# Quantco/tabmat

Hardware: AMD Instinct MI355X
Metric: SplitMatrix.sandwich GFLOP/s + effective HBM GB/s, 10M×1k mixed (higher is better)
Workload: dtype f64; 1 GPU; SplitMatrix.sandwich: dense128 + csr512@5% + cats(256,96,32), 10000000 rows/GPU, p=1024, float64 (BASELINE configs[3]); rows_per_gpu=10000000, p=1024, launch=eager, collective=none

## Files before the change

### tabmat_amd/csrc/cat_multi.hip

```cpp
#include <algorithm>
#include <type_traits>

#include "common.hpp"
#include "reduce.hpp"

namespace tmh {

constexpr int MAX_CATS = 16;
struct CatSet {
    const int32_t *codes[MAX_CATS];
    int ncol[MAX_CATS];
    int drop[MAX_CATS];
    int off[MAX_CATS];
    int n_cats;
    int total;
};

__host__ __device__ constexpr size_t tile_lds_bytes(size_t nel) { return ((nel * sizeof(lds_acc_t) + 15) / 16) * 16; }

__device__ __forceinline__ void zero_tile(lds_acc_t *tile, int nel) {
    for (int b = threadIdx.x; b < nel; b += blockDim.x) tile[b] = 0.0;
}

__device__ __forceinline__ unsigned char *scratch_behind_tile(unsigned char *smem, int nel) {
    return smem + tile_lds_bytes((size_t)nel);
}

template <typename F>
__device__ __forceinline__ F *workgroup_slice(F *ws, int64_t stride) {
    return ws + ((int64_t)blockIdx.y * gridDim.x + blockIdx.x) * stride;
}

template <typename F>
__device__ __forceinline__ void store_tile(const lds_acc_t *tile, int rows, int tstr, int cols, F *__restrict__ dst) {
    if (tstr == cols) {
        for (int b = threadIdx.x; b < rows * cols; b += blockDim.x) dst[b] = (F)tile[b];
    } else {
        for (int b = threadIdx.x; b < rows * cols; b += blockDim.x) dst[b] = (F)tile[(b / cols) * tstr + (b % cols)];
    }
}

__device__ __forceinline__ int level_of(const int32_t *codes, int drop, int64_t row) { return codes[row] - drop; }

constexpr int PACKED_BITS = 10;
constexpr int PACKED_NONE = (1 << PACKED_BITS) - 1;
__device__ __forceinline__ int packed_field(unsigned pk, int c) { return (int)((pk >> (PACKED_BITS * c)) & (unsigned)PACKED_NONE); }

template <typename F, int TJ, int NC>
__global__ __launch_bounds__(1024) void multi_cat_dense_c_kernel(
    CatSet cs, const F *__restrict__ d, const F *__restrict__ M, int64_t n, int64_t m,
    int64_t rows_per_block, F *__restrict__ ws, int64_t stride) {
    extern __shared__ __attribute__((aligned(16))) unsigned char smem_raw[];
    lds_acc_t *tile = reinterpret_cast<lds_acc_t *>(smem_raw);
    const int nel = cs.total * TJ;
    zero_tile(tile, nel);
    __syncthreads();
    constexpr int RPW = 64 / TJ;
    constexpr int UNR = 4;
    constexpr int NCC = NC > 0 ? NC : 1;
    const int lane = threadIdx.x & 63;
    const int sub = lane / TJ, jl = lane % TJ;
    const int wave = threadIdx.x >> 6, nwave = blockDim.x >> 6;
    const int64_t j = (int64_t)blockIdx.y * TJ + jl;
    const bool jok = j < m;
    const int64_t t0 = (int64_t)blockIdx.x * rows_per_block;
    const int64_t t1 = min(t0 + rows_per_block, n);
    const int64_t step = (int64_t)nwave * RPW;
    for (int64_t k0 = t0 + (int64_t)wave * RPW + sub; k0 < t1; k0 += UNR * step) {
        F x[UNR];
        int cc[UNR][NCC];
#pragma unroll
        for (int u = 0; u < UNR; ++u) {
            const int64_t k = k0 + u * step;
            const bool ok = k < t1;
            x[u] = (ok && jok) ? d[k] * M[k * m + j] : F(0);
            if (NC > 0) {
#pragma unroll
                for (int c = 0; c < NCC; ++c) cc[u][c] = ok ? level_of(cs.codes[c], cs.drop[c], k) : -1;
            }
        }
        if (NC > 0) {
#pragma unroll
            for (int u = 0; u < UNR; ++u)
#pragma unroll
                for (int c = 0; c < NCC; ++c)
                    if (jok && cc[u][c] >= 0)
                        atomic_add(&tile[(cs.off[c] + cc[u][c]) * TJ + jl], (lds_acc_t)x[u]);
        } else {
#pragma unroll 1
            for (int c = 0; c < cs.n_cats; ++c) {
#pragma unroll
                for (int u = 0; u < UNR; ++u) {
                    const int64_t k = k0 + u * step;
                    const int c1 = k < t1 ? level_of(cs.codes[c], cs.drop[c], k) : -1;
                    if (jok && c1 >= 0) atomic_add(&tile[(cs.off[c] + c1) * TJ + jl], (lds_acc_t)x[u]);
                }
            }
        }
    }
    __syncthreads();
    store_tile(tile, cs.total, TJ, TJ, workgroup_slice(ws, stride));
}

constexpr int MCW_RS = 32;
constexpr int MCW_VEC = 2;

template <typename F, int NC>
__global__ __launch_bounds__(1024) void multi_cat_dense_wide_kernel(
    CatSet cs, const F *__restrict__ d, const F *__restrict__ M, int64_t n, int64_t m,
    int64_t rows_per_block, F *__restrict__ ws, int64_t stride, const int32_t *__restrict__ rows,
    WgLogBuf *__restrict__ wglog) {
    const unsigned long long t_begin = wg_log_begin(wglog);
    constexpr int VEC = MCW_VEC;
    constexpr int TJ = 16 * VEC;
    constexpr int NI = MCW_RS / 4;
    typedef F vec_t __attribute__((ext_vector_type(VEC)));
    extern __shared__ __attribute__((aligned(16))) unsigned char smem_raw[];
    lds_acc_t *tile = reinterpret_cast<lds_acc_t *>(smem_raw);
    const int nel = cs.total * TJ;
    zero_tile(tile, nel);
    const int lane = threadIdx.x & 63;
    const int wave = threadIdx.x >> 6, nwave = blockDim.x >> 6;
    unsigned char *scr = scratch_behind_tile(smem_raw, nel) + (size_t)wave * MCW_RS * (sizeof(F) + NC * sizeof(int));
    F *sd = reinterpret_cast<F *>(scr);
    int *sc = reinterpret_cast<int *>(scr + MCW_RS * sizeof(F));
    __syncthreads();
    const int q = lane >> 4, jl = lane & 15;
    const int64_t j = (int64_t)blockIdx.y * TJ + jl * VEC;
    const int64_t jc = min(j, m - VEC);
    const bool jok = j < m;
    const int64_t t0 = (int64_t)blockIdx.x * rows_per_block;
    const int64_t t1 = min(t0 + rows_per_block, n);
    const int64_t step = (int64_t)nwave * MCW_RS;
    const int lr = lane & (MCW_RS - 1);

    struct Regs { vec_t x[NI]; F dk; int code[NC]; };
    auto load = [&](int64_t k0, Regs &R) {
        int64_t kr[NI];
#pragma unroll
        for (int i = 0; i < NI; ++i) kr[i] = min(k0 + 4 * i + q, n - 1);
        if (rows) {
#pragma unroll
            for (int i = 0; i < NI; ++i) kr[i] = (int64_t)rows[kr[i]];
        }
#pragma unroll
        for (int i = 0; i < NI; ++i) {
            R.x[i] = __builtin_nontemporal_load(reinterpret_cast<const vec_t *>(M + kr[i] * m + jc));
        }
        const int64_t k = k0 + lr;
        const int64_t kp = min(k, n - 1);
        const int64_t kc = rows ? (int64_t)rows[kp] : kp;
        R.dk = d[kc];
#pragma unroll
        for (int c = 0; c < NC; ++c) {
            const int col = level_of(cs.codes[c], cs.drop[c], kc);
            R.code[c] = (k < t1 && col >= 0) ? (cs.off[c] + col) * TJ * (int)sizeof(lds_acc_t) : -1;
        }
    };
    auto process = [&](const Regs &R) {
        __builtin_amdgcn_wave_barrier();
        if (lane < MCW_RS) {
            sd[lr] = R.dk;
#pragma unroll
            for (int c = 0; c < NC; ++c)
                sc[c * MCW_RS + lr] = R.dk != F(0) ? R.code[c] : -1;
        }
        __builtin_amdgcn_wave_barrier();
#pragma unroll
        for (int i = 0; i < NI; ++i) {
            const int row = 4 * i + q;
            const F dk = sd[row];
            int off[NC];
#pragma unroll
            for (int c = 0; c < NC; ++c) off[c] = sc[c * MCW_RS + row];
            vec_t x = R.x[i];
#pragma unroll
            for (int v = 0; v < VEC; ++v) x[v] *= dk;
#pragma unroll
            for (int c = 0; c < NC; ++c) {
                if (jok && off[c] >= 0) {
                    lds_acc_t *dst = reinterpret_cast<lds_acc_t *>(smem_raw + off[c]) + jl;
#pragma unroll
                    for (int v = 0; v < VEC; ++v) atomic_add(dst + 16 * v, (lds_acc_t)x[v]);
                }
            }
        }
    };
    Regs ra, rb;
    int64_t k0 = t0 + (int64_t)wave * MCW_RS;
    if (k0 < t1) load(k0, ra);
    for (; k0 < t1; k0 += 2 * step) {
        const bool more = k0 + step < t1;
        if (more) load(k0 + step, rb);
        process(ra);
        if (more) {
            if (k0 + 2 * step < t1) load(k0 + 2 * step, ra);
            process(rb);
        }
    }
    __syncthreads();
    if (threadIdx.x == 0) wg_log_end(wglog, t_begin, WG_CAT_DENSE);
    F *dst = workgroup_slice(ws, stride);
    for (int b = threadIdx.x; b < nel; b += blockDim.x) {
        const int c = b % TJ;
        dst[b] = (F)tile[(b / TJ) * TJ + (c / VEC) + 16 * (c % VEC)];
    }
}

template <typename F, int TJ>
__global__ __launch_bounds__(1024) void multi_cat_dense_f_kernel(
    CatSet cs, const F *__restrict__ d, const F *__restrict__ M, int64_t n, int64_t m,
    int64_t rows_per_block, F *__restrict__ ws, int64_t stride) {
    extern __shared__ __attribute__((aligned(16))) unsigned char smem_raw[];
    lds_acc_t *tile = reinterpret_cast<lds_acc_t *>(smem_raw);
    const int nel = cs.total * TJ;
    zero_tile(tile, nel);
    __syncthreads();
    const int64_t j0 = (int64_t)blockIdx.y * TJ;
    const int64_t t0 = (int64_t)blockIdx.x * rows_per_block;
    const int64_t t1 = min(t0 + rows_per_block, n);
    for (int64_t k = t0 + threadIdx.x; k < t1; k += blockDim.x) {
        const F dk = d[k];
        int col[MAX_CATS];
#pragma unroll
        for (int c = 0; c < MAX_CATS; ++c)
            col[c] = c < cs.n_cats ? level_of(cs.codes[c], cs.drop[c], k) : -1;
        for (int jl = 0; jl < TJ && j0 + jl < m; ++jl) {
            const F x = dk * M[(j0 + jl) * n + k];
#pragma unroll
            for (int c = 0; c < MAX_CATS; ++c)
                if (col[c] >= 0) atomic_add(&tile[(cs.off[c] + col[c]) * TJ + jl], (lds_acc_t)x);
        }
    }
    __syncthreads();
    store_tile(tile, cs.total, TJ, TJ, workgroup_slice(ws, stride));
}

template <typename F>
__global__ void multi_cat_untile_kernel(const F *__restrict__ tmp, int64_t total, int64_t m,
                                        int TJ, F *__restrict__ out) {
    const int64_t e = (int64_t)blockIdx.x * blockDim.x + threadIdx.x;
    if (e >= total * m) return;
    const int64_t a = e / m, j = e % m;
    out[e] = tmp[((j / TJ) * total + a) * TJ + (j % TJ)];
}

template <typename F, bool STAGE>
__global__ __launch_bounds__(1024) void multi_cat_sparse_kernel(
    CatSet cs, const F *__restrict__ d, const F *__restrict__ vals,
    const unsigned *__restrict__ koff, const unsigned char *__restrict__ ecol,
    const int64_t *__restrict__ gptr, int n_groups, int64_t n_slabs, int64_t slabs_per_block,
    int slab_rows, int group_cols, int64_t n, F *__restrict__ ws, int64_t stride) {
    extern __shared__ __attribute__((aligned(16))) unsigned char smem_raw[];
    lds_acc_t *tile = reinterpret_cast<lds_acc_t *>(smem_raw);
    const int tstr = group_cols + 1;
    const int nel = cs.total * tstr;
    zero_tile(tile, nel);
    const int g = blockIdx.y;
    const int lane = threadIdx.x & 63;
    const int wave = threadIdx.x >> 6, nwave = blockDim.x >> 6;
    unsigned char *scratch = scratch_behind_tile(smem_raw, nel);
    F *sd = reinterpret_cast<F *>(scratch) + (size_t)wave * slab_rows;
    int32_t *sc = reinterpret_cast<int32_t *>(reinterpret_cast<F *>(scratch) + (size_t)nwave * slab_rows) +
                  (size_t)wave * cs.n_cats * slab_rows;
    __syncthreads();
    const int64_t s0 = (int64_t)blockIdx.x * slabs_per_block;
    const int64_t s1 = min(s0 + slabs_per_block, n_slabs);
    const unsigned rowb = 64u * (unsigned)sizeof(F);
    int64_t nb = 0, ne = 0;
    if (s0 + wave < s1) {
        nb = gptr[(s0 + wave) * n_groups + g];
        ne = gptr[(s0 + wave) * n_groups + g + 1];
    }
    for (int64_t s = s0 + wave; s < s1; s += nwave) {
        const int64_t base = nb, end = ne;
        if (s + nwave < s1) {
            nb = gptr[(s + nwave) * n_groups + g];
            ne = gptr[(s + nwave) * n_groups + g + 1];
        }
        if (STAGE) {
            __builtin_amdgcn_wave_barrier();
            for (int r = lane; r < slab_rows; r += 64) {
                const int64_t k = min(s * slab_rows + r, n - 1);
                sd[r] = d[k];
                for (int c = 0; c < cs.n_cats; ++c) sc[c * slab_rows + r] = level_of(cs.codes[c], cs.drop[c], k);
            }
            __builtin_amdgcn_wave_barrier();
        }
        for (int64_t e0 = base + lane; e0 < end; e0 += 128) {
            const int64_t e1 = e0 + 64;
            const bool ok1 = e1 < end;
            const unsigned ko0 = koff[e0];
            const unsigned ko1 = ok1 ? koff[e1] : 0u;
            const F v0 = vals[e0];
            const F v1 = ok1 ? vals[e1] : F(0);
            const int ec0 = ecol[e0];
            const int ec1 = ok1 ? ecol[e1] : 0;
            const int r0 = (int)(ko0 / rowb), r1 = (int)(ko1 / rowb);
            const int64_t k0 = s * slab_rows + r0;
            const int64_t k1 = s * slab_rows + r1;
            const F d0 = STAGE ? sd[r0] : d[k0];
            const F d1 = ok1 ? (STAGE ? sd[r1] : d[k1]) : F(0);
            const F x0 = d0 != F(0) ? d0 * v0 : F(0);
            const F x1 = d1 != F(0) ? d1 * v1 : F(0);
#pragma unroll 1
            for (int c = 0; c < cs.n_cats; ++c) {
                const int c0 = STAGE ? sc[c * slab_rows + r0] : level_of(cs.codes[c], cs.drop[c], k0);
                const int c1 = ok1 ? (STAGE ? sc[c * slab_rows + r1] : level_of(cs.codes[c], cs.drop[c], k1)) : -1;
                if (c0 >= 0) atomic_add(&tile[(cs.off[c] + c0) * tstr + ec0], (lds_acc_t)x0);
                if (c1 >= 0) atomic_add(&tile[(cs.off[c] + c1) * tstr + ec1], (lds_acc_t)x1);
            }
        }
    }
    __syncthreads();
    store_tile(tile, cs.total, tstr, group_cols, workgroup_slice(ws, stride));
}

template <typename F, int NC>
__global__ __launch_bounds__(1024) void multi_cat_sparse_pf_kernel(
    CatSet cs, const F *__restrict__ d, const F *__restrict__ vals,
    const unsigned *__restrict__ koff, const unsigned char *__restrict__ ecol,
    const int64_t *__restrict__ gptr, int n_groups, int64_t n_slabs, int64_t slabs_per_block,
    int group_cols, int64_t n, F *__restrict__ ws, int64_t stride, WgLogBuf *__restrict__ wglog) {
    const unsigned long long t_begin = wg_log_begin(wglog);
    constexpr int SR = 128;
    constexpr int NQ = 4;
    extern __shared__ __attribute__((aligned(16))) unsigned char smem_raw[];
    lds_acc_t *tile = reinterpret_cast<lds_acc_t *>(smem_raw);
    const int tstr = group_cols + 1;
    const int nel = cs.total * tstr;
    zero_tile(tile, nel);
    const int g = blockIdx.y;
    const int lane = threadIdx.x & 63;
    const int wave = threadIdx.x >> 6, nwave = blockDim.x >> 6;
    unsigned char *scratch = scratch_behind_tile(smem_raw, nel);
    F *sd = reinterpret_cast<F *>(scratch) + (size_t)wave * SR;
    int32_t *sc = reinterpret_cast<int32_t *>(reinterpret_cast<F *>(scratch) + (size_t)nwave * SR) +
                  (size_t)wave * NC * SR;
    __syncthreads();
    const int64_t s0 = (int64_t)blockIdx.x * slabs_per_block;
    const int64_t s1 = min(s0 + slabs_per_block, n_slabs);
    const unsigned rowb = 64u * (unsigned)sizeof(F);

    int64_t q_base = 0, q_end = 0;
    int64_t p_base = 0, p_end = 0;
    unsigned p_ko[NQ];
    F p_v[NQ];
    int p_ec[NQ];
    F p_d[2];
    int p_c[NC][2];
    auto load_ptrs = [&](int64_t s) {
        q_base = q_end = 0;
        if (s < s1) {
            q_base = gptr[s * n_groups + g];
            q_end = gptr[s * n_groups + g + 1];
        }
    };
    auto load_block = [&](int64_t s) {
        p_base = q_base;
        p_end = q_end;
#pragma unroll
        for (int q = 0; q < NQ; ++q) {
            const int64_t e = p_base + q * 64 + lane;
            const int64_t ec = min(e, max(p_end - 1, p_base));
            const bool ok = e < p_end;
            p_ko[q] = ok ? koff[ec] : 0u;
            p_v[q] = ok ? vals[ec] : F(0);
            p_ec[q] = ok ? (int)ecol[ec] : 0;
        }
        if (s < s1) {
#pragma unroll
            for (int h = 0; h < 2; ++h) {
                const int64_t k = min(s * SR + lane + 64 * h, n - 1);
                p_d[h] = d[k];
#pragma unroll
                for (int c = 0; c < NC; ++c) p_c[c][h] = level_of(cs.codes[c], cs.drop[c], k);
            }
        }
    };
    const int64_t sw = s0 + wave;
    load_ptrs(sw);
    load_block(sw);
    load_ptrs(sw + nwave);
    for (int64_t s = sw; s < s1; s += nwave) {
        const int64_t base = p_base, end = p_end;
        unsigned ko[NQ];
        F v[NQ];
        int ec[NQ];
#pragma unroll
        for (int q = 0; q < NQ; ++q) { ko[q] = p_ko[q]; v[q] = p_v[q]; ec[q] = p_ec[q]; }
        __builtin_amdgcn_wave_barrier();
#pragma unroll
        for (int h = 0; h < 2; ++h) {
            sd[lane + 64 * h] = p_d[h];
#pragma unroll
            for (int c = 0; c < NC; ++c) sc[c * SR + lane + 64 * h] = p_c[c][h];
        }
        __builtin_amdgcn_wave_barrier();
        load_block(s + nwave);
        load_ptrs(s + 2 * nwave);
        auto scatter = [&](unsigned kk, F vv, int ee) {
            const int r = (int)(kk / rowb);
            const F dk = sd[r];
            const F x = dk != F(0) ? dk * vv : F(0);
#pragma unroll
            for (int c = 0; c < NC; ++c) {
                const int cc = sc[c * SR + r];
                if (cc >= 0) atomic_add(&tile[(cs.off[c] + cc) * tstr + ee], (lds_acc_t)x);
            }
        };
#pragma unroll
        for (int q = 0; q < NQ; ++q)
            if (base + q * 64 + lane < end) scatter(ko[q], v[q], ec[q]);
        for (int64_t e = base + NQ * 64 + lane; e < end; e += 64) scatter(koff[e], vals[e], (int)ecol[e]);
    }
    __syncthreads();
    if (threadIdx.x == 0) wg_log_end(wglog, t_begin, WG_CAT_SPARSE);
    store_tile(tile, cs.total, tstr, group_cols, workgroup_slice(ws, stride));
}

#ifndef EN_CS_U
#define EN_CS_U 4
#endif
template <typename F, int NC>
__global__ __launch_bounds__(1024) void multi_cat_sparse_ent_kernel(
    CatSet cs, const F *__restrict__ d, const F *__restrict__ vals, const unsigned short *__restrict__ meta,
    const unsigned *__restrict__ bstart, int n_groups, int64_t n, int64_t n_slabs, int64_t slabs_per_block,
    F *__restrict__ ws, int64_t stride, const unsigned *__restrict__ packed) {
    constexpr int GC = 32, TSTR = GC + 1;
    extern __shared__ __attribute__((aligned(16))) unsigned char smem_raw[];
    lds_acc_t *tile = reinterpret_cast<lds_acc_t *>(smem_raw);
    const int nel = cs.total * TSTR;
    zero_tile(tile, nel);
    __syncthreads();
    const int lane = threadIdx.x & 63;
    const int wave = threadIdx.x >> 6, nwave = blockDim.x >> 6;
    const int h = wave & 1;
    const int g = 2 * blockIdx.y + h;
    const int nwh = (nwave + 1 - h) / 2;
    const int wi = wave >> 1;
    const int64_t s0 = (int64_t)blockIdx.x * slabs_per_block;
    const int64_t s1 = min(s0 + slabs_per_block, n_slabs);
    if (g < n_groups && s1 > s0) {
        const int64_t spw = (s1 - s0 + nwh - 1) / nwh;
        const int64_t sa = min(s0 + (int64_t)wi * spw, s1), sb = min(sa + spw, s1);
        const unsigned *brow = bstart + (int64_t)g * (n_slabs + 1);
        const int64_t e0 = (int64_t)brow[sa] * 16, e1 = (int64_t)brow[sb] * 16;
        constexpr int U = EN_CS_U;
        struct Step { F v[U]; unsigned m[U]; F dk[U]; int c[U][NC]; };
        auto load_stream = [&](int64_t e, Step &t) {
#pragma unroll
            for (int u = 0; u < U; ++u) {
                const bool ok = e + 64 * u + lane < e1;
                const int64_t i = ok ? e + 64 * u + lane : (e1 > e0 ? e1 - 1 : 0);
                t.v[u] = ok ? vals[i] : F(0);
                t.m[u] = meta[i];
            }
        };
        unsigned cur_slab = (unsigned)sa;
        const unsigned row_max = (unsigned)(n - 1);
        auto load_rows = [&](Step &t) {
#pragma unroll
            for (int u = 0; u < U; ++u) {
                const unsigned slab = cur_slab + (((t.m[u] >> 10) - cur_slab) & 63u);
                cur_slab = (unsigned)__builtin_amdgcn_readlane((int)slab, 63);
                const unsigned row = min((slab << 6) | ((t.m[u] >> 4) & 63u), row_max);
                t.dk[u] = d[row];
                if (NC <= 3 && packed != nullptr) {
                    const unsigned pk = packed[row];
#pragma unroll
                    for (int c = 0; c < NC; ++c) {
                        const int f = packed_field(pk, c);
                        t.c[u][c] = f == PACKED_NONE ? -1 : f - cs.off[c];
                    }
                    continue;
                }
#pragma unroll
                for (int c = 0; c < NC; ++c) t.c[u][c] = level_of(cs.codes[c], cs.drop[c], row);
            }
        };
        if (e1 > e0) {
            Step cur, nxt, nx2;
            load_stream(e0, cur);
            load_stream(e0 + 64 * U, nxt);
            load_rows(cur);
            for (int64_t e = e0; e < e1; e += 64 * U) {
                load_stream(e + 128 * U, nx2);
                load_rows(nxt);
#pragma unroll
                for (int u = 0; u < U; ++u) {
                    const F x = (cur.dk[u] != F(0) && cur.v[u] != F(0)) ? cur.dk[u] * cur.v[u] : F(0);
                    const int col = 16 * h + (int)(cur.m[u] & 15u);
                    if (x != F(0)) {
#pragma unroll
                        for (int c = 0; c < NC; ++c)
                            if (cur.c[u][c] >= 0)
                                atomic_add(&tile[(cs.off[c] + cur.c[u][c]) * TSTR + col], (lds_acc_t)x);
                    }
                }
                cur = nxt;
                nxt = nx2;
            }
        }
    }
    __syncthreads();
    store_tile(tile, cs.total, TSTR, GC, workgroup_slice(ws, stride));
}

#ifndef EN_CS_D
#define EN_CS_D 4
#endif
#ifndef EN_CS_BOTH
#define EN_CS_BOTH 1
#endif
template <typename F, int NC, bool PK>
__global__ __launch_bounds__(1024) void multi_cat_sparse_ent_staged_kernel(
    CatSet cs, const F *__restrict__ d, const F *__restrict__ vals, const unsigned short *__restrict__ meta,
    const unsigned *__restrict__ bstart, int n_groups, int64_t n, int64_t n_slabs, int64_t slabs_per_block,
    F *__restrict__ ws, int64_t stride, const unsigned *__restrict__ packed, int tile_bytes) {
    constexpr int GC = 32, TSTR = GC + 1;
    constexpr int NCW = PK ? 1 : NC;
    extern __shared__ __attribute__((aligned(16))) unsigned char smem_raw[];
    lds_acc_t *tile = reinterpret_cast<lds_acc_t *>(smem_raw);
    const int nel = cs.total * TSTR;
    zero_tile(tile, nel);
    __syncthreads();
    const int lane = threadIdx.x & 63;
    const int wave = __builtin_amdgcn_readfirstlane(threadIdx.x >> 6), nwave = blockDim.x >> 6;
    F *sd = reinterpret_cast<F *>(smem_raw + tile_bytes) + wave * 64;
    int *sc = reinterpret_cast<int *>(smem_raw + tile_bytes + (size_t)nwave * 64 * sizeof(F)) + wave * 64 * NCW;
    constexpr int NG = EN_CS_BOTH ? 2 : 1;
    const int h0 = EN_CS_BOTH ? 0 : (wave & 1);
    const int g0 = 2 * blockIdx.y + h0;
    const int nwh = EN_CS_BOTH ? nwave : (nwave + 1 - h0) / 2;
    const int wi = EN_CS_BOTH ? wave : (wave >> 1);
    const int64_t s0 = (int64_t)blockIdx.x * slabs_per_block;
    const int64_t s1 = min(s0 + slabs_per_block, n_slabs);
    if (g0 < n_groups && s1 > s0) {
        const int64_t spw = (s1 - s0 + nwh - 1) / nwh;
        const int64_t sa = min(s0 + (int64_t)wi * spw, s1), sb = min(sa + spw, s1);
        const bool has[2] = {true, g0 + 1 < n_groups};
        const unsigned *brow[2] = {bstart + (int64_t)g0 * (n_slabs + 1),
                                   bstart + (int64_t)(has[1] ? g0 + 1 : g0) * (n_slabs + 1)};
        struct Bnd { unsigned b0[NG], b1[NG]; };
        struct Pre { F v[NG]; unsigned m[NG]; F dd; int c[NCW]; unsigned b0[NG]; int nsl[NG]; };
        int vz = 0;
#if defined(__HIP_DEVICE_COMPILE__)
        asm volatile("v_mov_b32 %0, 0" : "=v"(vz));
#endif
        auto request_bounds = [&](int64_t s, Bnd &q) {
            const int64_t sc_ = min(s, sb - 1) + vz;
#pragma unroll
            for (int k = 0; k < NG; ++k) {
                q.b0[k] = brow[k][sc_];
                q.b1[k] = brow[k][sc_ + 1];
            }
        };
        auto request = [&](int64_t s, const Bnd &q, Pre &p) {
            const bool live = s < sb;
#pragma unroll
            for (int k = 0; k < NG; ++k) {
                const unsigned qb0 = (unsigned)__builtin_amdgcn_readfirstlane((int)q.b0[k]);
                const unsigned qb1 = (unsigned)__builtin_amdgcn_readfirstlane((int)q.b1[k]);
                p.b0[k] = qb0;
                p.nsl[k] = (live && has[k]) ? (int)(qb1 - qb0) * 16 : 0;
                const bool ok = lane < p.nsl[k];
                const int64_t e = (int64_t)qb0 * 16 + (ok ? lane : 0);
                const F v = __builtin_nontemporal_load(vals + e);
                p.m[k] = __builtin_nontemporal_load(meta + e);
                p.v[k] = ok ? v : F(0);
            }
            const int64_t row_ = min(s, sb - 1) * 64 + lane;
            const int64_t row = min(row_, n - 1);
            p.dd = d[row];
            if constexpr (PK) {
                p.c[0] = (int)packed[row];
            } else {
#pragma unroll
                for (int c = 0; c < NC; ++c) p.c[c] = level_of(cs.codes[c], cs.drop[c], row);
            }
        };
        auto process = [&](Pre &p) {
            int any = 0;
#pragma unroll
            for (int k = 0; k < NG; ++k) any |= p.nsl[k];
            if (any == 0) return;
            sd[lane] = p.dd;
#pragma unroll
            for (int c = 0; c < NCW; ++c) sc[c * 64 + lane] = p.c[c];
            __builtin_amdgcn_wave_barrier();
#pragma unroll
            for (int k = 0; k < NG; ++k) {
                F v = p.v[k];
                unsigned m = p.m[k];
                const int cbase = 16 * (h0 + k);
                for (int off = 0; off < p.nsl[k]; off += 64) {
                    if (off > 0) {
                        const bool ok = off + lane < p.nsl[k];
                        const int64_t e = (int64_t)p.b0[k] * 16 + off + (ok ? lane : 0);
                        v = ok ? vals[e] : F(0);
                        m = meta[e];
                    }
                    const int r6 = (int)((m >> 4) & 63u);
                    const int col = cbase + (int)(m & 15u);
                    const F dk = sd[r6];
                    const F x = (dk != F(0) && v != F(0)) ? dk * v : F(0);
                    if (x != F(0)) {
                        if constexpr (PK) {
                            const unsigned pk = (unsigned)sc[r6];
#pragma unroll
                            for (int c = 0; c < NC; ++c) {
                                const int f = packed_field(pk, c);
                                if (f != PACKED_NONE) atomic_add(&tile[f * TSTR + col], (lds_acc_t)x);
                            }
                        } else {
#pragma unroll
                            for (int c = 0; c < NC; ++c) {
                                const int cc = sc[c * 64 + r6];
                                if (cc >= 0) atomic_add(&tile[(cs.off[c] + cc) * TSTR + col], (lds_acc_t)x);
                            }
                        }
                    }
                }
            }
            __builtin_amdgcn_wave_barrier();
        };
        constexpr int DEPTH = EN_CS_D;
        Pre p[DEPTH];
        Bnd q[DEPTH];
#pragma unroll
        for (int j = 0; j < DEPTH; ++j) request_bounds(sa + j, q[j]);
#pragma unroll
        for (int j = 0; j < DEPTH; ++j) {
            request(sa + j, q[j], p[j]);
            request_bounds(sa + DEPTH + j, q[j]);
        }
        for (int64_t s = sa; s < sb; s += DEPTH) {
#pragma unroll
            for (int j = 0; j < DEPTH; ++j) {
                process(p[j]);
                request(s + DEPTH + j, q[j], p[j]);
                request_bounds(s + 2 * DEPTH + j, q[j]);
            }
        }
    }
    __syncthreads();
    store_tile(tile, cs.total, TSTR, GC, workgroup_slice(ws, stride));
}

template <typename F, typename IX>
__global__ __launch_bounds__(1024) void multi_cat_sparse_rows_kernel(
    CatSet cs, const F *__restrict__ cm_data, const IX *__restrict__ cm_ind,
    const int32_t *__restrict__ ranges, const int32_t *__restrict__ rows, const F *__restrict__ d_sel,
    int64_t n_sel, int64_t rows_per_block, F *__restrict__ ws, int64_t stride) {
    constexpr int GC = 32;
    extern __shared__ __attribute__((aligned(16))) unsigned char smem_raw[];
    lds_acc_t *tile = reinterpret_cast<lds_acc_t *>(smem_raw);
    constexpr int tstr = GC + 1;
    const int nel = cs.total * tstr;
    zero_tile(tile, nel);
    __syncthreads();
    static_assert(SPARSE_CHUNK_COLS == 4 * GC, "the chunk of the chunk-major twin must hold four 32-column groups");
    const int g = blockIdx.y;
    const int ch = g >> 2;
    const int lane = threadIdx.x & 63, wave = threadIdx.x >> 6, nwave = blockDim.x >> 6;
    const int lr = lane >> 3, lt = lane & 7;
    const int64_t t0 = (int64_t)blockIdx.x * rows_per_block;
    const int64_t t1 = min(t0 + rows_per_block, n_sel);
    const int32_t *rg = ranges + (int64_t)ch * n_sel * 2;
    for (int64_t k0 = t0 + wave * 8; k0 < t1; k0 += (int64_t)nwave * 8) {
        const int64_t k = k0 + lr;
        if (k >= t1) continue;
        const F dk = d_sel[k];
        if (dk == F(0)) continue;
        const int e0 = rg[2 * k], e1 = rg[2 * k + 1];
        if (e0 >= e1) continue;
        const int64_t row = rows[k];
        int off[MAX_CATS];
#pragma unroll
        for (int c = 0; c < MAX_CATS; ++c) {
            off[c] = -1;
            if (c < cs.n_cats) {
                const int col = level_of(cs.codes[c], cs.drop[c], row);
                off[c] = col >= 0 ? (cs.off[c] + col) * tstr : -1;
            }
        }
        for (int e = e0 + lt; e < e1; e += 8) {
            const int col = (int)cm_ind[e] - (sizeof(IX) == 1 ? (g & 3) : g) * GC;
            if (col < 0 || col >= GC) continue;
            const lds_acc_t x = (lds_acc_t)(dk * cm_data[e]);
#pragma unroll
            for (int c = 0; c < MAX_CATS; ++c)
                if (off[c] >= 0) atomic_add(&tile[off[c] + col], x);
        }
    }
    __syncthreads();
    store_tile(tile, cs.total, tstr, GC, workgroup_slice(ws, stride));
}

__global__ __launch_bounds__(256) void multi_cat_pack_codes_kernel(CatSet cs, int64_t n, unsigned *__restrict__ out) {
    for (int64_t r = (int64_t)blockIdx.x * blockDim.x + threadIdx.x; r < n; r += (int64_t)gridDim.x * blockDim.x) {
        unsigned pk = 0u;
#pragma unroll
        for (int c = 0; c < 3; ++c) {
            unsigned f = (unsigned)PACKED_NONE;
            if (c < cs.n_cats) {
                const int col = level_of(cs.codes[c], cs.drop[c], r);
                if (col >= 0 && col < cs.ncol[c]) f = (unsigned)(cs.off[c] + col);
            }
            pk |= f << (PACKED_BITS * c);
        }
        out[r] = pk;
    }
}

constexpr size_t TILE_SCRATCH_LDS_MAX = 150 * 1024;
constexpr size_t ENT_STAGED_LDS_MAX = 156 * 1024;

static int make_catset(const void *const *h_codes, const int64_t *h_ncols, const int32_t *h_drop,
                       int n_cats, CatSet *cs) {
    if (n_cats < 1 || n_cats > MAX_CATS) {
        set_error("multi-cat call supports 1..%d categoricals, got %d", MAX_CATS, n_cats);
        return TM_EINVAL;
    }
    int off = 0;
    for (int c = 0; c < MAX_CATS; ++c) {
        cs->codes[c] = c < n_cats ? reinterpret_cast<const int32_t *>(h_codes[c]) : nullptr;
        cs->ncol[c] = c < n_cats ? (int)h_ncols[c] : 0;
        cs->drop[c] = c < n_cats ? h_drop[c] : 0;
        cs->off[c] = off;
        off += cs->ncol[c];
    }
    cs->n_cats = n_cats;
    cs->total = off;
    return TM_OK;
}

template <typename F>
static int fused_begin(const void *const *h_codes, const int64_t *h_ncols, const int32_t *h_drop, int n_cats,
                       int64_t units, int64_t m, F *out, hipStream_t st, CatSet *cs, bool *done) {
    *done = true;
    int rc = make_catset(h_codes, h_ncols, h_drop, n_cats, cs);
    if (rc) return rc;
    const int64_t total = (int64_t)cs->total * m;
    if (total == 0) return TM_OK;
    if (units == 0) {
        TM_HIP(hipMemsetAsync(out, 0, sizeof(F) * (size_t)total, st));
        return TM_OK;
    }
    *done = false;
    return TM_OK;
}

static int tile_fits(const char *what, const CatSet &cs, size_t tile_bytes) {
    if (tile_bytes <= HIST_LDS_MAX) return TM_OK;
    set_error("%s: %d stacked categories exceed the LDS tile", what, cs.total);
    return TM_EUNSUPPORTED;
}

struct RangeCut {
    int64_t nblk, per;
};
static RangeCut cut_ranges(int64_t units, int64_t parts, const char *rounds_knob, int64_t min_units, int64_t align) {
    const int64_t rounds = rounds_knob ? tune(rounds_knob, 1) : 1;
    int64_t nblk = std::max<int64_t>(1, rounds * NUM_CU / parts);
    nblk = std::min<int64_t>(nblk, std::max<int64_t>(1, ceil_div(units, min_units)));
    const int64_t per = ceil_div(ceil_div(units, nblk), align) * align;
    return {ceil_div(units, per), per};
}

template <typename F, typename Kern, typename Launch>
static int launch_and_finish(Kern kern, int64_t nblk, int64_t parts, int threads, size_t lds, const CatSet &cs,
                             int part_cols, int64_t m, F *out, hipStream_t st, Launch &&launch) {
    const int64_t stride = (int64_t)cs.total * part_cols;
    const size_t tmp_bytes = ((sizeof(F) * (size_t)(parts * stride) + 255) / 256) * 256;
    void *wsv = nullptr;
    int rc = get_workspace(tmp_bytes + sizeof(F) * (size_t)(parts * nblk * stride) + 256, &wsv, st);
    if (rc) return rc;
    F *tmp = reinterpret_cast<F *>(wsv);
    F *ws = reinterpret_cast<F *>(reinterpret_cast<char *>(wsv) + tmp_bytes);
    if (lds > 48 * 1024)
        TM_HIP(hipFuncSetAttribute(reinterpret_cast<const void *>(kern), hipFuncAttributeMaxDynamicSharedMemorySize,
                                   (int)lds));
    prof_begin(st);
    launch(dim3((unsigned)nblk, (unsigned)parts), dim3((unsigned)threads), ws, stride);
    prof_end(st);
    TM_LAUNCH_CHECK();
    rc = launch_reduce_partials<F>(ws, stride, (int)nblk, (int)parts, tmp, parts * stride, false, st);
    if (rc) return rc;
    hipLaunchKernelGGL((multi_cat_untile_kernel<F>), dim3((unsigned)ceil_div((int64_t)cs.total * m, 256)), dim3(256), 0,
                       st, tmp, (int64_t)cs.total, m, part_cols, out);
    TM_LAUNCH_CHECK();
    return TM_OK;
}

template <int MAX_NC, int OVER = MAX_NC, int NC = 1, typename Fn>
static int dispatch_nc(int n_cats, Fn &&f) {
    if constexpr (NC > MAX_NC) return f(std::integral_constant<int, OVER>{});
    else return n_cats == NC ? f(std::integral_constant<int, NC>{}) : dispatch_nc<MAX_NC, OVER, NC + 1>(n_cats, f);
}

template <int TJ = 64, typename Fn>
static int dispatch_tj(int tj, Fn &&f) {
    if (tj == TJ) return f(std::integral_constant<int, TJ>{});
    if constexpr (TJ > 1) return dispatch_tj<TJ / 2>(tj, f);
    return TM_EINVAL;
}

static int waves_knob(const char *knob, int dflt) {
    return (int)std::min<int64_t>(16, std::max<int64_t>(4, tune(knob, dflt)));
}

template <typename F>
static int run_multi_cat_dense(const void *const *h_codes, const int64_t *h_ncols,
                               const int32_t *h_drop, int n_cats, int64_t n, const F *d, const F *M,
                               int64_t m, int order_f, F *out, hipStream_t st,
                               const int32_t *rows = nullptr, int64_t n_rows = 0) {
    if (rows != nullptr) n = n_rows;
    CatSet cs;
    bool done;
    int rc = fused_begin(h_codes, h_ncols, h_drop, n_cats, n, m, out, st, &cs, &done);
    if (rc || done) return rc;
    constexpr int TJW = 16 * MCW_VEC;
    const size_t tile_b = tile_lds_bytes((size_t)cs.total * TJW);
    const size_t lds_w = tile_b + (size_t)16 * MCW_RS * (sizeof(F) + (size_t)n_cats * sizeof(int));
    if (!order_f && n_cats <= 8 && m >= MCW_VEC && m % MCW_VEC == 0 &&
        (reinterpret_cast<uintptr_t>(M) & 15) == 0 && lds_w <= TILE_SCRATCH_LDS_MAX &&
        (int64_t)cs.total * TJW * (int64_t)sizeof(lds_acc_t) < (1ll << 30)) {
        const int64_t n_parts = ceil_div(m, TJW);
        const RangeCut cut = cut_ranges(n, n_parts, "catdense_rounds", 4096, MCW_RS);
        const int nw = waves_knob("catdense_waves", (sizeof(F) == 8 && tile_b > 64 * 1024) ? 8 : 16);
        return dispatch_nc<8>(n_cats, [&](auto nc) {
            auto kern = &multi_cat_dense_wide_kernel<F, decltype(nc)::value>;
            auto launch = [&](dim3 grid, dim3 block, F *ws, int64_t stride) {
                hipLaunchKernelGGL(kern, grid, block, lds_w, st, cs, d, M, n, m, cut.per, ws, stride, rows, wg_log_ptr());
            };
            return launch_and_finish<F>(kern, cut.nblk, n_parts, nw * 64, lds_w, cs, TJW, m, out, st, launch);
        });
    }
    if (rows != nullptr) {
        set_error("multi_cat_dense: the row-list form needs the wide-load path");
        return TM_EUNSUPPORTED;
    }
    int TJ = 64;
    while (TJ > 1 && sizeof(lds_acc_t) * (size_t)cs.total * TJ > HIST_LDS_MAX) TJ >>= 1;
    while (TJ > 1 && TJ / 2 >= m) TJ >>= 1;
    const size_t lds = sizeof(lds_acc_t) * (size_t)cs.total * TJ;
    rc = tile_fits("multi_cat_dense", cs, lds);
    if (rc) return rc;
    const int64_t n_parts = ceil_div(m, TJ);
    const RangeCut cut = cut_ranges(n, n_parts, nullptr, 4096, 1);
    return dispatch_tj(TJ, [&](auto tj) {
        auto go = [&](auto kern) {
            auto launch = [&](dim3 grid, dim3 block, F *ws, int64_t stride) {
                hipLaunchKernelGGL(kern, grid, block, lds, st, cs, d, M, n, m, cut.per, ws, stride);
            };
            return launch_and_finish<F>(kern, cut.nblk, n_parts, 1024, lds, cs, TJ, m, out, st, launch);
        };
        constexpr int V = decltype(tj)::value;
        if (order_f) return go(&multi_cat_dense_f_kernel<F, V>);
        return dispatch_nc<4, 0>(n_cats, [&](auto nc) { return go(&multi_cat_dense_c_kernel<F, V, decltype(nc)::value>); });
    });
}

template <typename F>
static int run_multi_cat_sparse(const void *const *h_codes, const int64_t *h_ncols,
                                const int32_t *h_drop, int n_cats, int64_t n, const F *d,
                                const F *vals, const unsigned *koff, const unsigned char *ecol,
                                const int64_t *gptr, int64_t m, int slab_rows, int group_cols,
                                F *out, hipStream_t st) {
    CatSet cs;
    bool done;
    int rc = fused_begin(h_codes, h_ncols, h_drop, n_cats, n, m, out, st, &cs, &done);
    if (rc || done) return rc;
    const size_t tile_bytes = tile_lds_bytes((size_t)cs.total * (group_cols + 1));
    rc = tile_fits("multi_cat_sparse", cs, tile_bytes);
    if (rc) return rc;
    const int nw = waves_knob("catsparse_waves", 16);
    const size_t stage_bytes = (size_t)nw * slab_rows * (sizeof(F) + sizeof(int32_t) * (size_t)n_cats);
    const bool stage = tile_bytes + stage_bytes <= TILE_SCRATCH_LDS_MAX;
    const size_t lds = tile_bytes + (stage ? stage_bytes : 0);
    const int n_groups = (int)ceil_div(m, group_cols);
    const int64_t n_slabs = ceil_div(n, slab_rows);
    const RangeCut cut = cut_ranges(n_slabs, n_groups, "catsparse_rounds", 1, 1);
    if (stage && n_cats <= 8 && slab_rows == 128)
        return dispatch_nc<8>(n_cats, [&](auto nc) {
            auto kern = &multi_cat_sparse_pf_kernel<F, decltype(nc)::value>;
            auto launch = [&](dim3 grid, dim3 block, F *ws, int64_t stride) {
                hipLaunchKernelGGL(kern, grid, block, lds, st, cs, d, vals, koff, ecol, gptr, n_groups, n_slabs, cut.per,
                                   group_cols, n, ws, stride, wg_log_ptr());
            };
            return launch_and_finish<F>(kern, cut.nblk, n_groups, nw * 64, lds, cs, group_cols, m, out, st, launch);
        });
    auto kern = stage ? &multi_cat_sparse_kernel<F, true> : &multi_cat_sparse_kernel<F, false>;
    auto launch = [&](dim3 grid, dim3 block, F *ws, int64_t stride) {
        hipLaunchKernelGGL(kern, grid, block, lds, st, cs, d, vals, koff, ecol, gptr, n_groups, n_slabs, cut.per,
                           slab_rows, group_cols, n, ws, stride);
    };
    return launch_and_finish<F>(kern, cut.nblk, n_groups, nw * 64, lds, cs, group_cols, m, out, st, launch);
}

template <typename F>
static int run_multi_cat_sparse_ent(const void *const *h_codes, const int64_t *h_ncols, const int32_t *h_drop,
                                    int n_cats, int64_t n, const F *d, const F *vals, const unsigned short *meta,
                                    const unsigned *bstart, int64_t mk, F *out, hipStream_t st,
                                    const unsigned *packed = nullptr, int64_t n_slots = 0) {
    CatSet cs;
    bool done;
    int rc = fused_begin(h_codes, h_ncols, h_drop, n_cats, n, mk, out, st, &cs, &done);
    if (rc || done) return rc;
    TM_REQUIRE(mk % 16 == 0 && n_cats >= 1 && n_cats <= 8, "kernel columns in groups of 16, 1 .. 8 categoricals");
    TM_REQUIRE(n < (1ll << 28), "at most 2^28 - 1 rows per block");
    constexpr int GC = 32;
    const size_t lds = tile_lds_bytes((size_t)cs.total * (GC + 1));
    rc = tile_fits("multi_cat_sparse_ent", cs, lds);
    if (rc) return rc;
    TM_REQUIRE(packed == nullptr || (n_cats <= 3 && cs.total < PACKED_NONE), "packed codes: at most 3 categoricals, 1022 levels");
    const int nw = waves_knob("catsparse_waves", 16);
    const int n_groups = (int)(mk / 16);
    const int n_pairs = (n_groups + 1) / 2;
    const int64_t n_slabs = ceil_div(n, 64);
    const RangeCut cut = cut_ranges(n_slabs, n_pairs, "catsparse_rounds", 1, 1);
    auto finish = [&](auto kern, size_t lds_k, auto &&launch) {
        return launch_and_finish<F>(kern, cut.nblk, n_pairs, nw * 64, lds_k, cs, GC, mk, out, st, launch);
    };
    const int ncw = packed != nullptr ? 1 : n_cats;
    const size_t lds_staged = lds + (size_t)nw * 64 * (sizeof(F) + 4 * (size_t)ncw);
    const double fill = (double)n_slots / ((double)std::max(n_groups, 1) * (double)n_slabs);
    if (tune("catsparse_staged", 1) != 0 && lds_staged <= ENT_STAGED_LDS_MAX &&
        fill >= (double)tune("catsparse_staged_fill", 44)) {
        auto staged = [&](auto kern) {
            return finish(kern, lds_staged, [&](dim3 grid, dim3 block, F *ws, int64_t stride) {
                hipLaunchKernelGGL(kern, grid, block, lds_staged, st, cs, d, vals, meta, bstart, n_groups, n, n_slabs,
                                   cut.per, ws, stride, packed, (int)lds);
            });
        };
        if (packed != nullptr)
            return dispatch_nc<3>(n_cats, [&](auto nc) {
                return staged(&multi_cat_sparse_ent_staged_kernel<F, decltype(nc)::value, true>);
            });
        return dispatch_nc<8>(n_cats, [&](auto nc) {
            return staged(&multi_cat_sparse_ent_staged_kernel<F, decltype(nc)::value, false>);
        });
    }
    return dispatch_nc<8>(n_cats, [&](auto nc) {
        auto kern = &multi_cat_sparse_ent_kernel<F, decltype(nc)::value>;
        return finish(kern, lds, [&](dim3 grid, dim3 block, F *ws, int64_t stride) {
            hipLaunchKernelGGL(kern, grid, block, lds, st, cs, d, vals, meta, bstart, n_groups, n, n_slabs, cut.per, ws,
                               stride, packed);
        });
    });
}

template <typename F, typename IX>
static int run_multi_cat_sparse_rows(const void *const *h_codes, const int64_t *h_ncols,
                                     const int32_t *h_drop, int n_cats, const F *cm_data,
                                     const IX *cm_ind, const int32_t *ranges, const int32_t *rows,
                                     int64_t n_sel, int64_t m, const F *d_sel, F *out, hipStream_t st) {
    CatSet cs;
    bool done;
    int rc = fused_begin(h_codes, h_ncols, h_drop, n_cats, n_sel, m, out, st, &cs, &done);
    if (rc || done) return rc;
    constexpr int GC = 32;
    const size_t lds = tile_lds_bytes((size_t)cs.total * (GC + 1));
    rc = tile_fits("multi_cat_sparse_rows", cs, lds);
    if (rc) return rc;
    const int n_groups = (int)ceil_div(m, GC);
    const RangeCut cut = cut_ranges(n_sel, n_groups, "catsparse_rounds", 2048, 1);
    auto kern = &multi_cat_sparse_rows_kernel<F, IX>;
    auto launch = [&](dim3 grid, dim3 block, F *ws, int64_t stride) {
        hipLaunchKernelGGL(kern, grid, block, lds, st, cs, cm_data, cm_ind, ranges, rows, d_sel, n_sel, cut.per, ws, stride);
    };
    return launch_and_finish<F>(kern, cut.nblk, n_groups, 1024, lds, cs, GC, m, out, st, launch);
}

}

using namespace tmh;


extern "C" {

int tm_multi_cat_dense_sandwich_f32(const void *const *h_codes, const int64_t *h_ncols,
                                    const int32_t *h_drop_first, int n_cats, int64_t n,
                                    const float *d, const float *M, int64_t M_ncol, int order_f,
                                    float *out, void *stream) {
    return run_multi_cat_dense<float>(h_codes, h_ncols, h_drop_first, n_cats, n, d, M, M_ncol,
                                      order_f, out, as_stream(stream));
}
int tm_multi_cat_dense_sandwich_f64(const void *const *h_codes, const int64_t *h_ncols,
                                    const int32_t *h_drop_first, int n_cats, int64_t n,
                                    const double *d, const double *M, int64_t M_ncol, int order_f,
                                    double *out, void *stream) {
    return run_multi_cat_dense<double>(h_codes, h_ncols, h_drop_first, n_cats, n, d, M, M_ncol,
                                       order_f, out, as_stream(stream));
}
int tm_multi_cat_dense_sandwich_rows_f32(const void *const *h_codes, const int64_t *h_ncols,
                                         const int32_t *h_drop_first, int n_cats, int64_t n,
                                         const float *d, const float *M, int64_t M_ncol,
                                         const int32_t *rows, int64_t n_rows, float *out,
                                         void *stream) {
    return run_multi_cat_dense<float>(h_codes, h_ncols, h_drop_first, n_cats, n, d, M, M_ncol, 0, out,
                                      as_stream(stream), rows, n_rows);
}
int tm_multi_cat_dense_sandwich_rows_f64(const void *const *h_codes, const int64_t *h_ncols,
                                         const int32_t *h_drop_first, int n_cats, int64_t n,
                                         const double *d, const double *M, int64_t M_ncol,
                                         const int32_t *rows, int64_t n_rows, double *out,
                                         void *stream) {
    return run_multi_cat_dense<double>(h_codes, h_ncols, h_drop_first, n_cats, n, d, M, M_ncol, 0, out,
                                       as_stream(stream), rows, n_rows);
}
int tm_multi_cat_sparse_sandwich_ent_f32(const void *const *h_codes, const int64_t *h_ncols,
                                         const int32_t *h_drop_first, int n_cats, int64_t n, const float *d,
                                         const float *vals, const uint16_t *meta, const uint32_t *bstart,
                                         int64_t n_slots, int64_t mk, float *out, void *stream) {
    return run_multi_cat_sparse_ent<float>(h_codes, h_ncols, h_drop_first, n_cats, n, d, vals, meta, bstart, mk,
                                           out, as_stream(stream), nullptr, n_slots);
}
int tm_multi_cat_sparse_sandwich_ent_f64(const void *const *h_codes, const int64_t *h_ncols,
                                         const int32_t *h_drop_first, int n_cats, int64_t n, const double *d,
                                         const double *vals, const uint16_t *meta, const uint32_t *bstart,
                                         int64_t n_slots, int64_t mk, double *out, void *stream) {
    return run_multi_cat_sparse_ent<double>(h_codes, h_ncols, h_drop_first, n_cats, n, d, vals, meta, bstart, mk,
                                            out, as_stream(stream), nullptr, n_slots);
}
int tm_multi_cat_pack_codes(const void *const *h_codes, const int64_t *h_ncols, const int32_t *h_drop_first, int n_cats,
                            int64_t n, uint32_t *packed, void *stream) {
    CatSet cs;
    int rc = make_catset(h_codes, h_ncols, h_drop_first, n_cats, &cs);
    if (rc) return rc;
    TM_REQUIRE(n_cats <= 3 && cs.total < PACKED_NONE, "packed codes: at most 3 categoricals, 1022 stacked levels");
    if (n == 0) return TM_OK;
    hipLaunchKernelGGL(multi_cat_pack_codes_kernel, dim3((unsigned)std::min<int64_t>(4 * NUM_CU, ceil_div(n, 256))),
                       dim3(256), 0, as_stream(stream), cs, n, packed);
    TM_LAUNCH_CHECK();
    return TM_OK;
}
int tm_multi_cat_sparse_sandwich_entp_f32(const void *const *h_codes, const int64_t *h_ncols,
                                          const int32_t *h_drop_first, int n_cats, int64_t n, const float *d,
                                          const float *vals, const uint16_t *meta, const uint32_t *bstart,
                                          int64_t n_slots, int64_t mk, const uint32_t *packed, float *out, void *stream) {
    return run_multi_cat_sparse_ent<float>(h_codes, h_ncols, h_drop_first, n_cats, n, d, vals, meta, bstart, mk, out,
                                           as_stream(stream), packed, n_slots);
}
int tm_multi_cat_sparse_sandwich_entp_f64(const void *const *h_codes, const int64_t *h_ncols,
                                          const int32_t *h_drop_first, int n_cats, int64_t n, const double *d,
                                          const double *vals, const uint16_t *meta, const uint32_t *bstart,
                                          int64_t n_slots, int64_t mk, const uint32_t *packed, double *out, void *stream) {
    return run_multi_cat_sparse_ent<double>(h_codes, h_ncols, h_drop_first, n_cats, n, d, vals, meta, bstart, mk,
                                            out, as_stream(stream), packed, n_slots);
}
int tm_multi_cat_sparse_sandwich_slab_f32(const void *const *h_codes, const int64_t *h_ncols,
                                          const int32_t *h_drop_first, int n_cats, int64_t n,
                                          const float *d, const float *vals, const uint32_t *koff,
                                          const uint8_t *ecol, const int64_t *gptr, int64_t m,
                                          float *out, void *stream) {
    return run_multi_cat_sparse<float>(h_codes, h_ncols, h_drop_first, n_cats, n, d, vals, koff,
                                       ecol, gptr, m, tm_slab_rows(), tm_slab_group_cols(), out,
                                       as_stream(stream));
}
int tm_multi_cat_sparse_sandwich_slab_f64(const void *const *h_codes, const int64_t *h_ncols,
                                          const int32_t *h_drop_first, int n_cats, int64_t n,
                                          const double *d, const double *vals, const uint32_t *koff,
                                          const uint8_t *ecol, const int64_t *gptr, int64_t m,
                                          double *out, void *stream) {
    return run_multi_cat_sparse<double>(h_codes, h_ncols, h_drop_first, n_cats, n, d, vals, koff,
                                        ecol, gptr, m, tm_slab_rows(), tm_slab_group_cols(), out,
                                        as_stream(stream));
}
int tm_multi_cat_sparse_sandwich_rows_f32(const void *const *h_codes, const int64_t *h_ncols,
                                          const int32_t *h_drop_first, int n_cats,
                                          const float *cm_data, const int32_t *cm_indices,
                                          const int32_t *row_ranges, const int32_t *rows,
                                          int64_t n_sel, int64_t m, const float *d_sel, float *out,
                                          void *stream) {
    return run_multi_cat_sparse_rows<float, int32_t>(h_codes, h_ncols, h_drop_first, n_cats, cm_data,
                                                 cm_indices, row_ranges, rows, n_sel, m, d_sel, out,
                                                 as_stream(stream));
}
int tm_multi_cat_sparse_sandwich_rows_f64(const void *const *h_codes, const int64_t *h_ncols,
                                          const int32_t *h_drop_first, int n_cats,
                                          const double *cm_data, const int32_t *cm_indices,
                                          const int32_t *row_ranges, const int32_t *rows,
                                          int64_t n_sel, int64_t m, const double *d_sel, double *out,
                                          void *stream) {
    return run_multi_cat_sparse_rows<double, int32_t>(h_codes, h_ncols, h_drop_first, n_cats, cm_data,
                                                  cm_indices, row_ranges, rows, n_sel, m, d_sel, out,
                                                  as_stream(stream));
}
int tm_multi_cat_sparse_sandwich_rows_u8_f32(const void *const *h_codes, const int64_t *h_ncols,
                                             const int32_t *h_drop_first, int n_cats,
                                             const float *cm_data, const uint8_t *cm_col8,
                                             const int32_t *row_ranges, const int32_t *rows,
                                             int64_t n_sel, int64_t m, const float *d_sel, float *out,
                                             void *stream) {
    return run_multi_cat_sparse_rows<float, uint8_t>(h_codes, h_ncols, h_drop_first, n_cats, cm_data,
                                                          cm_col8, row_ranges, rows, n_sel, m, d_sel, out,
                                                          as_stream(stream));
}
int tm_multi_cat_sparse_sandwich_rows_u8_f64(const void *const *h_codes, const int64_t *h_ncols,
                                             const int32_t *h_drop_first, int n_cats,
                                             const double *cm_data, const uint8_t *cm_col8,
                                             const int32_t *row_ranges, const int32_t *rows,
                                             int64_t n_sel, int64_t m, const double *d_sel, double *out,
                                             void *stream) {
    return run_multi_cat_sparse_rows<double, uint8_t>(h_codes, h_ncols, h_drop_first, n_cats, cm_data,
                                                           cm_col8, row_ranges, rows, n_sel, m, d_sel, out,
                                                           as_stream(stream));
}
}
```

### tabmat_amd/csrc/reduce.hpp

```cpp
#pragma once
#include "common.hpp"

namespace tmh {

template <typename F, bool ACCUMULATE, int NW>
__global__ __launch_bounds__(NW * 64) void reduce_partials_kernel(const F *__restrict__ ws,
                                                                  int64_t stride, int nb,
                                                                  F *__restrict__ out,
                                                                  int64_t out_elems) {
    __shared__ double red[NW][64];
    const int lane = threadIdx.x & 63;
    const int wave = threadIdx.x >> 6;
    const int64_t e = (int64_t)blockIdx.x * 64 + lane;
    const int part = blockIdx.y;
    double acc = 0.0;
    if (e < stride) {
        const F *p = ws + ((int64_t)part * nb) * stride + e;
        for (int b = wave; b < nb; b += NW) acc += (double)p[(int64_t)b * stride];
    }
    red[wave][lane] = acc;
    __syncthreads();
    if (wave == 0 && e < stride) {
        const int64_t o = (int64_t)part * stride + e;
        if (o < out_elems) {
            double s = 0.0;
#pragma unroll
            for (int w = 0; w < NW; w += 4)
                s += (red[w][lane] + red[w + 1][lane]) + (red[w + 2][lane] + red[w + 3][lane]);
            if (ACCUMULATE)
                out[o] += (F)s;
            else
                out[o] = (F)s;
        }
    }
}

template <typename F>
inline int launch_reduce_partials(const F *ws, int64_t stride, int nb, int n_parts, F *out,
                                  int64_t out_elems, bool accumulate, hipStream_t st) {
    dim3 grid((unsigned)ceil_div(stride, 64), (unsigned)n_parts);
    const bool small = (int64_t)grid.x * grid.y < 1024 && nb > 16;
    if (small) {
        if (accumulate)
            hipLaunchKernelGGL((reduce_partials_kernel<F, true, 16>), grid, dim3(1024), 0, st, ws,
                               stride, nb, out, out_elems);
        else
            hipLaunchKernelGGL((reduce_partials_kernel<F, false, 16>), grid, dim3(1024), 0, st, ws,
                               stride, nb, out, out_elems);
    } else if (accumulate) {
        hipLaunchKernelGGL((reduce_partials_kernel<F, true, 4>), grid, dim3(256), 0, st, ws, stride,
                           nb, out, out_elems);
    } else {
        hipLaunchKernelGGL((reduce_partials_kernel<F, false, 4>), grid, dim3(256), 0, st, ws, stride,
                           nb, out, out_elems);
    }
    TM_LAUNCH_CHECK();
    return TM_OK;
}

__global__ void fill_i32_kernel(int32_t *p, int64_t n, int32_t v);
__global__ void scatter_iota_i32_kernel(int32_t *map, const int32_t *cols, int64_t n_cols);

int build_col_map(int32_t *map, int64_t m, const int32_t *cols, int64_t n_cols, hipStream_t st);

}
```

### tabmat_amd/csrc/sparse_blocks.hip

```cpp
#include <algorithm>

#include "common.hpp"
#include "reduce.hpp"

namespace tmh {

constexpr int KB_WAVES = 16;
constexpr int KB_TS = 128;

template <typename F>
__global__ void blocks_assemble_kernel(const F *__restrict__ tiles, int n_out, F *__restrict__ out) {
    const int j = blockIdx.x * blockDim.x + threadIdx.x;
    const int i = blockIdx.y;
    if (i >= n_out || j >= n_out) return;
    const int hi = max(i, j), lo = min(i, j);
    const int I = hi / KB_TS, J = lo / KB_TS;
    const int part = I * (I + 1) / 2 + J;
    out[(int64_t)i * n_out + j] = tiles[(int64_t)part * KB_TS * KB_TS + (hi % KB_TS) * KB_TS + (lo % KB_TS)];
}

constexpr int KB_FLAG_REP_A = 1 << 16;
constexpr int KB_FLAG_REP_B = 1 << 17;

template <typename F, bool U8, bool D12 = false>
__global__ __launch_bounds__(KB_WAVES * 64) void sparse_sandwich_blocks_kernel(
    const F *__restrict__ data, const int32_t *__restrict__ ind, const int32_t *__restrict__ cptr,
    int64_t n, int64_t nnz1, const int32_t *__restrict__ blocks, const int4 *__restrict__ wg_tab,
    const F *__restrict__ d, int max_nb, F *__restrict__ ws, WgLogBuf *__restrict__ wglog) {
    constexpr int TS = KB_TS;
    const unsigned long long t_begin = wg_log_begin(wglog);
    extern __shared__ __attribute__((aligned(16))) unsigned char smem_raw[];
    lds_acc_t *tile = reinterpret_cast<lds_acc_t *>(smem_raw);
    const int4 w = wg_tab[2 * blockIdx.x], x = wg_tab[2 * blockIdx.x + 1];
    const int part = __builtin_amdgcn_readfirstlane(w.x), slot = __builtin_amdgcn_readfirstlane(w.y);
    const int b0 = __builtin_amdgcn_readfirstlane(w.z), b1 = __builtin_amdgcn_readfirstlane(w.w);
    const int bfull = __builtin_amdgcn_readfirstlane(x.x);
    int wfull = __builtin_amdgcn_readfirstlane(x.y);
    {
        const int nwv = (int)(blockDim.x >> 6);
        if (nwv != KB_WAVES) {
            wfull = (wfull * nwv + KB_WAVES / 2) / KB_WAVES;
            if (bfull > b0) wfull = max(wfull, 1);
            if (b1 > bfull) wfull = min(wfull, nwv - 1);
            if (bfull == b0) wfull = 0;
            if (b1 == bfull) wfull = nwv;
        }
    }
    int I = (int)((sqrtf(8.0f * (float)part + 1.0f) - 1.0f) * 0.5f);
    while ((I + 1) * (I + 2) / 2 <= part) ++I;
    while (I * (I + 1) / 2 > part) --I;
    const int J = part - I * (I + 1) / 2;
    const int i0 = I * TS, j0 = J * TS;
    for (int b = threadIdx.x; b < TS * TS; b += blockDim.x) tile[b] = 0.0;
    __syncthreads();

    const int lane = threadIdx.x & 63;
    const int wave = __builtin_amdgcn_readfirstlane(threadIdx.x >> 6);
    const int lr = lane >> 3, lt = lane & 7;
    if (b1 > b0) {
        const int row_first = __builtin_amdgcn_readfirstlane(x.z), row_last = __builtin_amdgcn_readfirstlane(x.w);
        const int32_t *cpA = cptr + (int64_t)I * (n + 1), *cpB = cptr + (int64_t)J * (n + 1);
        const int baseA = __builtin_amdgcn_readfirstlane(cpA[row_first]);
        const int baseB = __builtin_amdgcn_readfirstlane(cpB[row_first]);
        const unsigned spanA1 = (unsigned)max(__builtin_amdgcn_readfirstlane(cpA[row_last + 1]) - baseA - 1, 0);
        const unsigned spanB1 = (unsigned)max(__builtin_amdgcn_readfirstlane(cpB[row_last + 1]) - baseB - 1, 0);
        const F *dataA = data + min((int64_t)baseA, nnz1), *dataB = data + min((int64_t)baseB, nnz1);
        const int32_t *indA = ind + min((int64_t)baseA, nnz1), *indB = ind + min((int64_t)baseB, nnz1);
        const unsigned char *ind8 = reinterpret_cast<const unsigned char *>(ind);
        const unsigned char *ind8A = ind8 + min((int64_t)baseA, nnz1), *ind8B = ind8 + min((int64_t)baseB, nnz1);
        const int i0c = U8 ? 0 : i0, j0c = U8 ? 0 : j0;
        const unsigned nrow1 = (unsigned)max(n - 1, (int64_t)0);
        auto ldi = [](const int32_t *base, unsigned i) {
            return *reinterpret_cast<const int32_t *>(reinterpret_cast<const char *>(base) + (i << 2));
        };
        auto ldf = [](const F *base, unsigned i) {
            return *reinterpret_cast<const F *>(reinterpret_cast<const char *>(base) + (i * (unsigned)sizeof(F)));
        };
        constexpr int SH = 3;
        constexpr int BIGKEY = 0x7ffffff0;
        char *const tile_bytes = reinterpret_cast<char *>(tile);
        auto add_pair = [&](int kb, int la, int ba, F prod) {
            if (kb <= la)
                atomic_add(reinterpret_cast<lds_acc_t *>(tile_bytes + (unsigned)(kb ^ ba)), (lds_acc_t)prod);
        };

        auto run_list = [&](auto diag_c, auto full_c, int s0, int s1, int w0, int nw) {
            constexpr bool DIAG = decltype(diag_c)::value;
            constexpr bool FULL = decltype(full_c)::value;
            constexpr int offmask = DIAG ? 0 : 0x70000000;
            const int nseg = s1 - s0;
            if (nseg <= 0) return;
            constexpr int DW = D12 ? 3 : 4;
            const int32_t *blk = blocks + (int64_t)s0 * DW;
            struct Dsc { int4 q; bool valid; };
            struct Grp { int nA, nB, ta, tb; F d, va, vb; int ca, cb; };
            auto load_desc = [&](int g) {
                Dsc r;
                const int k = g + lr;
                r.valid = k < nseg;
                const unsigned kc = (unsigned)min(k, nseg - 1);
                if constexpr (D12) {
                    const int32_t *b = reinterpret_cast<const int32_t *>(reinterpret_cast<const char *>(blk) + kc * 12u);
                    const int x = b[0], y = b[1];
                    const unsigned w = (unsigned)b[2];
                    r.q = int4{x, y, (int)(w & 0xffffffu),
                               (int)((((w >> 24) & 7u) + 1u) | ((((w >> 27) & 7u) + 1u) << 8) | (((w >> 30) & 3u) << 16))};
                } else {
                    r.q = *reinterpret_cast<const int4 *>(reinterpret_cast<const char *>(blk) + (kc << 4));
                }
                return r;
            };
            auto load_entries = [&](const Dsc &sd) {
                Grp e;
                const unsigned row = min((unsigned)sd.q.z, nrow1);
                e.d = ldf(d, row);
                const bool on = sd.valid && e.d != F(0);
                e.nA = on ? (sd.q.w & 0xff) : 0;
                e.nB = on ? ((sd.q.w >> 8) & 0xff) : 0;
                e.ta = (!FULL && (sd.q.w & KB_FLAG_REP_A)) ? (lt & 3) : lt;
                e.tb = (!FULL && (sd.q.w & KB_FLAG_REP_B)) ? (lt & 3) : lt;
                const unsigned iA = min((unsigned)(sd.q.x - baseA) + min((unsigned)e.ta, (unsigned)max(e.nA - 1, 0)), spanA1);
                const unsigned iB = min((unsigned)(sd.q.y - baseB) + min((unsigned)e.tb, (unsigned)max(e.nB - 1, 0)), spanB1);
#ifdef KB_ABL_WRAP
                const unsigned iAw = iA & (unsigned)(KB_ABL_WRAP), iBw = iB & (unsigned)(KB_ABL_WRAP);
                e.ca = ldi(indA, min(iAw, spanA1));
                e.va = ldf(dataA, min(iAw, spanA1));
                e.cb = ldi(indB, min(iBw, spanB1));
                e.vb = ldf(dataB, min(iBw, spanB1));
                return e;
#endif
                e.ca = U8 ? (int)ind8A[iA] : ldi(indA, iA);
                e.va = ldf(dataA, iA);
                e.cb = U8 ? (int)ind8B[iB] : ldi(indB, iB);
                e.vb = ldf(dataB, iB);
                return e;
            };
            auto process = [&](const Grp &cur) {
                __builtin_amdgcn_s_setprio(1);
                const int colA = cur.ta < cur.nA ? cur.ca - i0c : -1;
                const int colB = cur.tb < cur.nB ? cur.cb - j0c : -1;
                const int la = (colA < 0 ? -8 : colA << SH) | offmask;
                const int ba = (int)(((unsigned)colA << (7 + SH)) | ((colA & 15) << (3 + SH)));
                const int kb = colB < 0 ? BIGKEY : colB << SH;
                const F av = cur.va * cur.d, vb = cur.vb;
                add_pair(kb, la, ba, av * vb);
                add_pair(dpp_xor_i32<1>(kb), la, ba, av * dpp_xor<1>(vb));
                add_pair(dpp_xor_i32<2>(kb), la, ba, av * dpp_xor<2>(vb));
                add_pair(dpp_xor_i32<3>(kb), la, ba, av * dpp_xor<3>(vb));
#ifndef KB_ABL_HALFSTEPS
                if constexpr (FULL) {
                    const int kb4 = dpp_xor_i32<4>(kb);
                    const F vb4 = dpp_xor<4>(vb);
                    add_pair(kb4, la, ba, av * vb4);
                    add_pair(dpp_xor_i32<1>(kb4), la, ba, av * dpp_xor<1>(vb4));
                    add_pair(dpp_xor_i32<2>(kb4), la, ba, av * dpp_xor<2>(vb4));
                    add_pair(dpp_xor_i32<3>(kb4), la, ba, av * dpp_xor<3>(vb4));
                }
#endif
                __builtin_amdgcn_s_setprio(0);
            };
            const int gstep = nw * 8;
            const int gw = (wave - w0) * 8;
            Grp ea[2], eb[2];
            Dsc ps[2];
            ea[0] = load_entries(load_desc(gw));
            ea[1] = load_entries(load_desc(gw + gstep));
            ps[0] = load_desc(gw + 2 * gstep);
            ps[1] = load_desc(gw + 3 * gstep);
            for (int g = gw; g < nseg; g += 4 * gstep) {
                eb[0] = load_entries(ps[0]);
                eb[1] = load_entries(ps[1]);
                ps[0] = load_desc(g + 4 * gstep);
                ps[1] = load_desc(g + 5 * gstep);
                process(ea[0]);
                if (g + gstep < nseg) process(ea[1]);
                if (g + 2 * gstep >= nseg) break;
                ea[0] = load_entries(ps[0]);
                ea[1] = load_entries(ps[1]);
                ps[0] = load_desc(g + 6 * gstep);
                ps[1] = load_desc(g + 7 * gstep);
                process(eb[0]);
                if (g + 3 * gstep < nseg) process(eb[1]);
            }
        };
        auto run_tile = [&](auto diag_c) {
            if (wave < wfull) run_list(diag_c, std::true_type{}, b0, bfull, 0, wfull);
            else run_list(diag_c, std::false_type{}, bfull, b1, wfull, (int)(blockDim.x >> 6) - wfull);
        };
        if (I == J) run_tile(std::true_type{});
        else run_tile(std::false_type{});
    }
    __syncthreads();
    if (threadIdx.x == 0) wg_log_end(wglog, t_begin, WG_K2);
    F *dst = ws + ((int64_t)part * max_nb + slot) * (TS * TS);
    for (int b = threadIdx.x; b < TS * TS; b += blockDim.x) {
        const int r = b / TS, c = b % TS;
        dst[b] = (F)tile[r * TS + (c ^ ((r & 15) << 3))];
    }
}

template <typename F, bool U8 = false, bool D12 = false>
static int run_sparse_sandwich_blocks(const F *data, const int32_t *ind, const int32_t *cptr, int64_t n,
                                      int64_t m, int64_t nnz, const int32_t *blocks, const int32_t *wg_tab,
                                      int n_wg, int max_nb, const F *d, F *out, hipStream_t st) {
    if (m == 0) return TM_OK;
    if (n == 0 || nnz == 0 || n_wg == 0) {
        TM_HIP(hipMemsetAsync(out, 0, sizeof(F) * (size_t)(m * m), st));
        return TM_OK;
    }
    constexpr int TS = KB_TS;
    const int nchunk = (int)ceil_div(m, TS);
    const int n_parts = nchunk * (nchunk + 1) / 2;
    TM_REQUIRE(nnz < (1ll << 31) && n < (1ll << 29), "sparse block too large for the block-list sandwich");
    TM_REQUIRE(!D12 || n < (1ll << 24), "12-byte block descriptors hold 24 bits of row");
    TM_REQUIRE(max_nb >= 1 && n_wg >= 1, "empty workgroup table");
    const size_t lds = sizeof(lds_acc_t) * (size_t)(TS * TS);
    const size_t tmp_bytes = (sizeof(F) * (size_t)n_parts * TS * TS + 255) / 256 * 256;
    const size_t ws_bytes = sizeof(F) * (size_t)n_parts * (size_t)max_nb * TS * TS;
    void *wsv = nullptr;
    int rc = get_workspace(tmp_bytes + ws_bytes + 256, &wsv, st);
    if (rc) return rc;
    F *tmp = reinterpret_cast<F *>(wsv);
    F *ws = reinterpret_cast<F *>(reinterpret_cast<char *>(wsv) + tmp_bytes);
    TM_HIP(hipMemsetAsync(ws, 0, ws_bytes, st));
    auto kern = &sparse_sandwich_blocks_kernel<F, U8, D12>;
    TM_HIP(hipFuncSetAttribute(reinterpret_cast<const void *>(kern),
                               hipFuncAttributeMaxDynamicSharedMemorySize, (int)lds));
    prof_begin(st);
    const int kb_waves = (int)std::min<int64_t>(KB_WAVES, std::max<int64_t>(2, tune("k2b_waves", KB_WAVES)));
    hipLaunchKernelGGL(kern, dim3((unsigned)n_wg), dim3(kb_waves * 64), lds, st, data, ind, cptr, n, nnz - 1,
                       blocks, reinterpret_cast<const int4 *>(wg_tab), d,
                       max_nb, ws, wg_log_ptr());
    prof_end(st);
    TM_LAUNCH_CHECK();
    rc = launch_reduce_partials<F>(ws, (int64_t)TS * TS, max_nb, n_parts, tmp, (int64_t)n_parts * TS * TS,
                                   false, st);
    if (rc) return rc;
    hipLaunchKernelGGL((blocks_assemble_kernel<F>), dim3((unsigned)ceil_div(m, 64), (unsigned)m), dim3(64),
                       0, st, tmp, (int)m, out);
    TM_LAUNCH_CHECK();
    return TM_OK;
}

}

extern "C" {

int tm_sparse_sandwich_blocks_f32(const float *cm_data, const int32_t *cm_indices, const int32_t *cptr,
                                  int64_t n, int64_t m, int64_t nnz, const int32_t *blocks,
                                  const int32_t *wg_tab, int n_wg, int max_nb, const float *d, float *out,
                                  void *stream) {
    return tmh::run_sparse_sandwich_blocks<float>(cm_data, cm_indices, cptr, n, m, nnz, blocks, wg_tab, n_wg,
                                                  max_nb, d, out, tmh::as_stream(stream));
}
int tm_sparse_sandwich_blocks_f64(const double *cm_data, const int32_t *cm_indices, const int32_t *cptr,
                                  int64_t n, int64_t m, int64_t nnz, const int32_t *blocks,
                                  const int32_t *wg_tab, int n_wg, int max_nb, const double *d, double *out,
                                  void *stream) {
    return tmh::run_sparse_sandwich_blocks<double>(cm_data, cm_indices, cptr, n, m, nnz, blocks, wg_tab, n_wg,
                                                   max_nb, d, out, tmh::as_stream(stream));
}

int tm_sparse_sandwich_blocks_u8_f32(const float *cm_data, const uint8_t *cm_col8, const int32_t *cptr,
                                     int64_t n, int64_t m, int64_t nnz, const int32_t *blocks,
                                     const int32_t *wg_tab, int n_wg, int max_nb, const float *d, float *out,
                                     void *stream) {
    return tmh::run_sparse_sandwich_blocks<float, true>(cm_data, reinterpret_cast<const int32_t *>(cm_col8), cptr, n, m,
                                                        nnz, blocks, wg_tab, n_wg, max_nb, d, out,
                                                        tmh::as_stream(stream));
}
int tm_sparse_sandwich_blocks_u8_f64(const double *cm_data, const uint8_t *cm_col8, const int32_t *cptr,
                                     int64_t n, int64_t m, int64_t nnz, const int32_t *blocks,
                                     const int32_t *wg_tab, int n_wg, int max_nb, const double *d, double *out,
                                     void *stream) {
    return tmh::run_sparse_sandwich_blocks<double, true>(cm_data, reinterpret_cast<const int32_t *>(cm_col8), cptr, n, m,
                                                         nnz, blocks, wg_tab, n_wg, max_nb, d, out,
                                                         tmh::as_stream(stream));
}

int tm_sparse_sandwich_blocks_p12_f32(const float *cm_data, const uint8_t *cm_col8, const int32_t *cptr,
                                      int64_t n, int64_t m, int64_t nnz, const int32_t *blocks12,
                                      const int32_t *wg_tab, int n_wg, int max_nb, const float *d, float *out,
                                      void *stream) {
    return tmh::run_sparse_sandwich_blocks<float, true, true>(cm_data, reinterpret_cast<const int32_t *>(cm_col8), cptr,
                                                              n, m, nnz, blocks12, wg_tab, n_wg, max_nb, d, out,
                                                              tmh::as_stream(stream));
}
int tm_sparse_sandwich_blocks_p12_f64(const double *cm_data, const uint8_t *cm_col8, const int32_t *cptr,
                                      int64_t n, int64_t m, int64_t nnz, const int32_t *blocks12,
                                      const int32_t *wg_tab, int n_wg, int max_nb, const double *d, double *out,
                                      void *stream) {
    return tmh::run_sparse_sandwich_blocks<double, true, true>(cm_data, reinterpret_cast<const int32_t *>(cm_col8), cptr,
                                                               n, m, nnz, blocks12, wg_tab, n_wg, max_nb, d, out,
                                                               tmh::as_stream(stream));
}

}
```

### tabmat_amd/csrc/sparse_ent.hip

```cpp
#include "common.hpp"
#include "reduce.hpp"

namespace tmh {

constexpr int EN_R = 64;
constexpr int EN_C = 16;
constexpr int EN_NW = 16;
constexpr int EN_THREADS = EN_NW * 64;
constexpr int EN_W = 128;
constexpr int EN_B = 16;
constexpr int EN_SB = 64;

template <typename F>
struct EnLds {
    static constexpr int ROWB = EN_W * (int)sizeof(F);
    static constexpr int SLABB = EN_R * ROWB;
    static constexpr int SCR_OFF = ROWB + 2 * SLABB;
    static constexpr int CS_OFF = SCR_OFF + EN_NW * EN_SB * 16;
    static constexpr int TOTAL = CS_OFF + EN_NW * EN_C * (int)sizeof(double);
};

constexpr int EN_CVGPR = 24;
#define EN_LD "40"

#if defined(__HIP_DEVICE_COMPILE__)
typedef __amdgpu_buffer_rsrc_t en_rsrc_t;
__device__ __forceinline__ en_rsrc_t en_rsrc(const void *base, int64_t bytes) {
    const unsigned nb = bytes <= 0 ? 0u : (bytes > 0xFFFFFFFFll ? 0xFFFFFFFFu : (unsigned)bytes);
    return __builtin_amdgcn_make_buffer_rsrc(const_cast<void *>(base), 0, (int)nb, 0x00020000);
}
__device__ __forceinline__ void en_buf_to_lds16(en_rsrc_t rs, void *lds, int voff, int soff) {
    __builtin_amdgcn_raw_ptr_buffer_load_lds(rs, (__attribute__((address_space(3))) void *)lds, 16, voff,
                                             soff, 0, 0);
}
template <typename F>
__device__ __forceinline__ void en_zero_acc() {
    if constexpr (sizeof(F) == 8) {
        static_for<16>([&](auto jc) {
            asm volatile("v_mov_b32 v[64+4*%0], 0\n\tv_mov_b32 v[64+4*%0+1], 0\n\t"
                         "v_mov_b32 v[64+4*%0+2], 0\n\tv_mov_b32 v[64+4*%0+3], 0"
                         :: "n"(decltype(jc)::value) : "v127");
        });
    } else {
        static_for<16>([&](auto jc) {
            asm volatile("v_mov_b32 v[64+2*%0], 0\n\tv_mov_b32 v[64+2*%0+1], 0" :: "n"(decltype(jc)::value) : "v95");
        });
    }
}
template <int K>
__device__ __forceinline__ unsigned en_read_acc() {
    unsigned x;
    asm volatile("v_mov_b32 %0, v[64+%1]" : "=v"(x) : "n"(K));
    return x;
}
template <typename F>
__device__ __forceinline__ void en_load_stream(unsigned voff_v, const F *vp, unsigned voff_m, const unsigned short *mp) {
    if constexpr (sizeof(F) == 8)
        asm volatile("global_load_dwordx2 v[" EN_LD ":" EN_LD "+1], %0, %1\n\t"
                     "global_load_ushort v[" EN_LD "+2], %2, %3" :: "v"(voff_v), "s"(vp), "v"(voff_m), "s"(mp) : "memory");
    else
        asm volatile("global_load_dword v[" EN_LD "], %0, %1\n\t"
                     "global_load_ushort v[" EN_LD "+2], %2, %3" :: "v"(voff_v), "s"(vp), "v"(voff_m), "s"(mp) : "memory");
}
template <typename F>
__device__ __forceinline__ void en_load_d(unsigned voff, const F *dp) {
    if constexpr (sizeof(F) == 8)
        asm volatile("global_load_dwordx2 v[" EN_LD "+4:" EN_LD "+5], %0, %1" :: "v"(voff), "s"(dp) : "memory");
    else
        asm volatile("global_load_dword v[" EN_LD "+4], %0, %1" :: "v"(voff), "s"(dp) : "memory");
}
template <int N>
__device__ __forceinline__ void en_take(double &v, unsigned &m, double &dd) {
    unsigned vl, vh, dl, dh;
    asm volatile("s_waitcnt vmcnt(%5)\n\t"
                 "v_mov_b32 %0, v[" EN_LD "]\n\tv_mov_b32 %1, v[" EN_LD "+1]\n\tv_mov_b32 %2, v[" EN_LD "+2]\n\t"
                 "v_mov_b32 %3, v[" EN_LD "+4]\n\tv_mov_b32 %4, v[" EN_LD "+5]"
                 : "=v"(vl), "=v"(vh), "=v"(m), "=v"(dl), "=v"(dh) : "n"(N) : "memory");
    v = __hiloint2double((int)vh, (int)vl);
    dd = __hiloint2double((int)dh, (int)dl);
}
template <int N>
__device__ __forceinline__ void en_take(float &v, unsigned &m, float &dd) {
    unsigned vl, dl;
    asm volatile("s_waitcnt vmcnt(%3)\n\t"
                 "v_mov_b32 %0, v[" EN_LD "]\n\tv_mov_b32 %1, v[" EN_LD "+2]\n\tv_mov_b32 %2, v[" EN_LD "+4]"
                 : "=v"(vl), "=v"(m), "=v"(dl) : "n"(N) : "memory");
    v = __uint_as_float(vl);
    dd = __uint_as_float(dl);
}
#else
struct en_rsrc_t {};
__device__ inline en_rsrc_t en_rsrc(const void *, int64_t) { return {}; }
__device__ inline void en_buf_to_lds16(en_rsrc_t, void *, int, int) {}
template <typename F> __device__ void en_zero_acc() {}
template <int K> __device__ unsigned en_read_acc() { return 0u; }
template <typename F> __device__ void en_load_stream(unsigned, const F *, unsigned, const unsigned short *) {}
template <typename F> __device__ void en_load_d(unsigned, const F *) {}
template <int N, typename F> __device__ void en_take(F &, unsigned &, F &) {}
#endif

template <int N, typename F>
__device__ __forceinline__ void en_batch_asm(unsigned &p0, unsigned &p1, unsigned &p2, unsigned &p3, F a, unsigned kq,
                                             unsigned lane_off);
#if defined(__HIP_DEVICE_COMPILE__)
#include "sparse_ent_batch.inc"
#else
template <int N, typename F>
__device__ void en_batch_asm(unsigned &, unsigned &, unsigned &, unsigned &, F, unsigned, unsigned) {}
#endif

template <typename F, bool CSUM>
__global__ __launch_bounds__(EN_THREADS) __attribute__((amdgpu_num_vgpr(EN_CVGPR))) void csr_dense_ent_kernel(
    const F *__restrict__ vals, const unsigned short *__restrict__ meta, const unsigned *__restrict__ bstart,
    int n_groups, int64_t n_slabs, int64_t slabs_per_block, const F *__restrict__ B, int64_t n, int64_t r,
    int nB, const F *__restrict__ d, F *__restrict__ ws, F *__restrict__ ws_csum, long long *__restrict__ prof) {
    extern __shared__ __attribute__((aligned(16))) unsigned char smem_raw[];
    using L = EnLds<F>;
    constexpr int ROWB = L::ROWB;
    constexpr int SLABB = L::SLABB;
    constexpr int NV = SLABB / 16 / EN_THREADS;
    constexpr int RPP = 1024 / ROWB;
    constexpr int RSH = sizeof(F) == 8 ? 10 : 9;
    constexpr int JSH = sizeof(F) == 8 ? 2 : 1;
    typedef __attribute__((address_space(3))) unsigned char lds_byte;
    typedef unsigned u4 __attribute__((ext_vector_type(4)));
    const int tid = threadIdx.x;
    const int lane = tid & 63;
    const int l16 = lane & 15;
    const int wave = __builtin_amdgcn_readfirstlane(tid >> 6);
    const int group = blockIdx.z * EN_NW + wave;
    const bool active = group < n_groups;
    const int j0 = blockIdx.y * EN_W;
    const int64_t s0 = (int64_t)blockIdx.x * slabs_per_block;
    const int ns = (int)(min(s0 + slabs_per_block, n_slabs) - s0);
    const unsigned lane_off = (unsigned)lane * 16u / (sizeof(F) == 8 ? 1u : 2u);
    const unsigned lds_base = (unsigned)(uintptr_t)(lds_byte *)smem_raw;
    u4 *scratch = reinterpret_cast<u4 *>(smem_raw + L::SCR_OFF) + wave * EN_SB;
    double *cs_lds = reinterpret_cast<double *>(smem_raw + L::CS_OFF) + wave * EN_C;

    en_zero_acc<F>();
    for (int i = tid; i < ROWB / 4; i += EN_THREADS) reinterpret_cast<unsigned *>(smem_raw)[i] = 0u;
    if (CSUM && lane < EN_C) cs_lds[lane] = 0.0;
    if (ns <= 0) return;

    constexpr int VEC = 16 / (int)sizeof(F);
    const int cc = min(j0 + ((lane * 16) % ROWB) / (int)sizeof(F), nB - VEC);
    const int row0 = wave * NV * RPP + (lane * 16) / ROWB;
    const unsigned boff0 = (unsigned)((row0 * r + cc) * (int64_t)sizeof(F));
    const int64_t pstride = (int64_t)RPP * r * (int64_t)sizeof(F);
    const int64_t bstride = (int64_t)EN_R * r * (int64_t)sizeof(F);
    const char *bnext = reinterpret_cast<const char *>(B) + s0 * bstride;
    int64_t bleft = n * r * (int64_t)sizeof(F) - s0 * bstride;
    auto issue_pieces = [&](int buf, int lo, int hi) {
#if defined(EN_ABL_NOCOPY)
        if (bnext != reinterpret_cast<const char *>(B) + s0 * bstride) return;
#endif
#pragma unroll
        for (int i = 0; i < NV; ++i)
            if (i >= lo && i < hi)
            en_buf_to_lds16(en_rsrc(bnext, bleft), smem_raw + ROWB + buf * SLABB + (wave * NV + i) * RPP * ROWB,
                            (int)boff0, (int)(i * pstride));
    };

    const unsigned *brow = bstart + (int64_t)(active ? group : 0) * (n_slabs + 1);
    const unsigned b0 = active ? brow[s0] : 0u;
    const int nbw = active ? (int)(brow[s0 + ns] - b0) : 0;
    const F *vbase = vals + (int64_t)b0 * EN_B;
    const unsigned short *mbase = meta + (int64_t)b0 * EN_B;
    F vx = F(0), vy = F(0), dy = F(0);
    unsigned mx = 0u, my = 0u;
    const unsigned lane_v = (unsigned)lane * (unsigned)sizeof(F), lane_m = (unsigned)lane * 2u;
    auto request_stream = [&](int k) {
        en_load_stream<F>(lane_v, vbase + (int64_t)k * EN_SB, lane_m, mbase + (int64_t)k * EN_SB);
    };
    const unsigned s0u = (unsigned)s0;
    unsigned cur_slab = s0u;
    auto expand = [&](unsigned m16) -> unsigned {
        const unsigned slab = cur_slab + (((m16 >> 10) - cur_slab) & 63u);
        cur_slab = (unsigned)__builtin_amdgcn_readlane((int)slab, 63);
        return (slab << 10) | (m16 & 0x3ffu);
    };
    const unsigned row_max = (unsigned)(n - 1);
    auto request_d = [&]() {
        en_load_d<F>(min(my >> 4, row_max) * (unsigned)sizeof(F), d);
    };
    auto wait_loads = [&](auto nc) { en_take<decltype(nc)::value>(vx, mx, dy); };
    int psince = 0;
    int lsince = 0;
    (void)lsince;
    auto boundary = [&](int k) {
        if (psince == 0) wait_loads(std::integral_constant<int, 0>{});
        else if (psince < NV) wait_loads(std::integral_constant<int, NV / 2>{});
        else if (psince < 2 * NV) wait_loads(std::integral_constant<int, NV>{});
        else wait_loads(std::integral_constant<int, 2 * NV>{});
        const unsigned rowg = my >> 4;
        const unsigned srel = (rowg >> 6) - s0u;
        const bool ok = vy != F(0) && dy != F(0);
        const F a = ok ? vy * dy : F(0);
        const unsigned kq = ok ? lds_base + (srel & 1u) * (unsigned)SLABB + (((rowg & 63u) + 1u) << RSH) : lds_base;
        const unsigned jv = (my & 15u) << JSH;
        const unsigned j1 = (unsigned)__builtin_amdgcn_update_dpp(0, (int)jv, 0x101, 0xf, 0xf, true);
        const unsigned j2 = (unsigned)__builtin_amdgcn_update_dpp(0, (int)jv, 0x102, 0xf, 0xf, true);
        const unsigned j3 = (unsigned)__builtin_amdgcn_update_dpp(0, (int)jv, 0x103, 0xf, 0xf, true);
        const unsigned jvs = (lane & 3) == 0 ? (jv | (j1 << 8) | (j2 << 16) | (j3 << 24)) : srel;
        u4 e;
        if constexpr (sizeof(F) == 8) {
            e = u4{(unsigned)__double2loint(a), (unsigned)__double2hiint(a), kq, jvs};
        } else {
            e = u4{__float_as_uint(a), 0u, kq, jvs};
        }
        scratch[lane] = e;
        if constexpr (CSUM) {
            if (4 * k * EN_B + lane < nbw * EN_B) atomic_add(cs_lds + (jv >> JSH), (double)a);
        }
        vy = vx;
        my = expand(mx);
        request_d();
        request_stream(k + 2);
        psince = 0;
        lsince += 3;
    };
    issue_pieces(0, 0, NV);
    bnext += bstride;
    bleft -= bstride;
    request_stream(0);
    wait_loads(std::integral_constant<int, 0>{});
    vy = vx;
    my = expand(mx);
    request_d();
    request_stream(1);
    __syncthreads();

#if defined(EN_PROF)
    long long pt_a = 0, pt_p = 0, pt_x = 0, pt_b = 0, pt_bar = 0, pt_n = 0;
    long long pt0 = clock64();
    const long long pt_start = pt0;
#define EN_TICK(acc) { const long long t_ = clock64(); acc += t_ - pt0; pt0 = t_; }
#else
#define EN_TICK(acc)
#endif
    int w = 0;
    int ncopied = 0;
    auto end_slab = [&]() {
        const bool more = w + 1 < ns;
        if (more) {
            if (ncopied < NV) {
                issue_pieces((w & 1) ^ 1, ncopied, NV);
                psince += NV - ncopied;
                lsince = 0;
            }
            bnext += bstride;
            bleft -= bstride;
        }
        EN_TICK(pt_p)
#if defined(EN_ABL_NOBARRIER)
#define EN_BAR ""
#else
#define EN_BAR "\n\ts_barrier"
#endif
#if defined(__HIP_DEVICE_COMPILE__)
        if (lsince == 0) asm volatile("s_waitcnt vmcnt(0) lgkmcnt(0)" EN_BAR ::: "memory");
        else if (lsince == 3) asm volatile("s_waitcnt vmcnt(3) lgkmcnt(0)" EN_BAR ::: "memory");
        else asm volatile("s_waitcnt vmcnt(6) lgkmcnt(0)" EN_BAR ::: "memory");
#endif
        EN_TICK(pt_bar)
        ncopied = 0;
        ++w;
    };
    u4 enext = u4{0u, 0u, 0u, 0u};
    for (int b = 0; b < nbw; ++b) {
        const int q = b & 3;
        u4 e;
        if (q == 0) {
            boundary(b >> 2);
            e = scratch[l16];
        } else {
            e = enext;
        }
        if (q != 3) enext = scratch[(q + 1) * EN_B + l16];
        EN_TICK(pt_a)
        const int slab = __builtin_amdgcn_readlane((int)e[3], 1);
        while (w < slab) end_slab();
        if (ncopied == 0 && w + 1 < ns) {
            issue_pieces((w & 1) ^ 1, 0, NV);

            ncopied = NV;
            psince += NV;
            lsince = 0;
        }
        EN_TICK(pt_p)
        F a;
        if constexpr (sizeof(F) == 8) a = __hiloint2double((int)e[1], (int)e[0]);
        else a = __uint_as_float(e[0]);
#if defined(EN_ABL_NOBATCH)
        asm volatile("" ::"v"(a), "v"(e[2]), "v"(e[3]));
#else
        const unsigned live = (unsigned)__builtin_amdgcn_ballot_w64(a != F(0)) & 0xffffu;
        const int nq = live ? ((31 - __builtin_clz(live)) >> 2) + 1 : 0;
        unsigned p0 = (unsigned)__builtin_amdgcn_readlane((int)e[3], 0);
        unsigned p1 = (unsigned)__builtin_amdgcn_readlane((int)e[3], 4);
        unsigned p2 = (unsigned)__builtin_amdgcn_readlane((int)e[3], 8);
        unsigned p3 = (unsigned)__builtin_amdgcn_readlane((int)e[3], 12);
        if (nq == 4) en_batch_asm<16, F>(p0, p1, p2, p3, a, e[2], lane_off);
        else if (nq == 3) en_batch_asm<12, F>(p0, p1, p2, p3, a, e[2], lane_off);
        else if (nq == 2) en_batch_asm<8, F>(p0, p1, p2, p3, a, e[2], lane_off);
        else if (nq == 1) en_batch_asm<4, F>(p0, p1, p2, p3, a, e[2], lane_off);
#endif
        EN_TICK(pt_x)
#if defined(EN_PROF)
        ++pt_n;
#endif
    }
    while (w < ns) end_slab();
    wait_loads(std::integral_constant<int, 0>{});
#if defined(EN_PROF)
    if (prof != nullptr && lane == 0) {
        long long *o = prof + (((int64_t)blockIdx.z * gridDim.y + blockIdx.y) * gridDim.x + blockIdx.x) * (EN_NW * 8) + wave * 8;
        o[0] = pt_a; o[1] = pt_p; o[2] = pt_x; o[3] = pt_b; o[4] = pt_bar; o[5] = pt_n; o[6] = clock64() - pt_start; o[7] = ns;
    }
#endif

    if (active) {
        F *dst = ws + (((int64_t)blockIdx.y * gridDim.x + blockIdx.x) * n_groups + group) * (EN_C * EN_W);
        static_for<EN_C>([&](auto jc) {
            constexpr int j = decltype(jc)::value;
            if constexpr (sizeof(F) == 8) {
                const u4 o = u4{en_read_acc<4 * j>(), en_read_acc<4 * j + 1>(), en_read_acc<4 * j + 2>(),
                                en_read_acc<4 * j + 3>()};
                *reinterpret_cast<u4 *>(dst + j * EN_W + 2 * lane) = o;
            } else {
                typedef unsigned u2 __attribute__((ext_vector_type(2)));
                const u2 o = u2{en_read_acc<2 * j>(), en_read_acc<2 * j + 1>()};
                *reinterpret_cast<u2 *>(dst + j * EN_W + 2 * lane) = o;
            }
        });
        if constexpr (CSUM) {
            if (blockIdx.y == 0 && lane < EN_C)
                ws_csum[(int64_t)blockIdx.x * (n_groups * EN_C) + group * EN_C + lane] = (F)cs_lds[lane];
        }
    }
}

template <typename F>
__global__ void en_untile_kernel(const F *__restrict__ tmp, int64_t m, int64_t nB, F *__restrict__ out) {
    const int64_t e = (int64_t)blockIdx.x * blockDim.x + threadIdx.x;
    if (e >= m * nB) return;
    const int64_t i = e / nB, j = e % nB;
    out[e] = tmp[((j / EN_W) * m + i) * EN_W + (j % EN_W)];
}

template <typename F>
__global__ void en_csum_kernel(const F *__restrict__ part, int nblk, int64_t m, F *__restrict__ csum) {
    const int64_t c = (int64_t)blockIdx.x * blockDim.x + threadIdx.x;
    if (c >= m) return;
    double a = 0.0;
    for (int b = 0; b < nblk; ++b) a += (double)part[(int64_t)b * m + c];
    csum[c] = (F)a;
}

template <typename F>
static int run_csr_dense_ent(const F *vals, const uint16_t *meta, const uint32_t *bstart, int64_t n, int64_t m,
                             const F *B, int64_t r, const F *d, F *out, F *colsum, hipStream_t st) {
    const int64_t nB = r;
    const int64_t total = m * nB;
    if (total == 0) return TM_OK;
    constexpr int VEC = 16 / (int)sizeof(F);
    if ((reinterpret_cast<uintptr_t>(B) & 15) != 0 || r % VEC != 0 || nB < VEC) {
        set_error("tm_csr_dense_sandwich_ent: B must be C-ordered with 16-byte aligned rows");
        return TM_EUNSUPPORTED;
    }
    if (m % EN_C != 0) {
        set_error("tm_csr_dense_sandwich_ent: m must be a multiple of tm_ent_group_cols()");
        return TM_EINVAL;
    }
    if (n >= (1ll << 28)) {
        set_error("tm_csr_dense_sandwich_ent: at most 2^28 - 1 rows per block (work in row parts)");
        return TM_EUNSUPPORTED;
    }
    const int64_t n_slabs = ceil_div(n, EN_R);
    const int n_groups = (int)(m / EN_C);
    const int n_parts = (int)ceil_div(nB, EN_W);
    const int nz = (int)ceil_div(n_groups, EN_NW);
    const bool want_csum = colsum != nullptr;
    if (n_slabs == 0) {
        TM_HIP(hipMemsetAsync(out, 0, sizeof(F) * (size_t)total, st));
        if (want_csum) TM_HIP(hipMemsetAsync(colsum, 0, sizeof(F) * (size_t)m, st));
        return TM_OK;
    }
    int64_t nblk = std::max<int64_t>(1, tune("ent_rounds", 1) * NUM_CU / ((int64_t)n_parts * nz));
    nblk = std::min<int64_t>(nblk, n_slabs);
    const int64_t spb = ceil_div(n_slabs, nblk);
    nblk = ceil_div(n_slabs, spb);
    const int64_t stride = m * EN_W;
    const size_t tmp_bytes = (sizeof(F) * (size_t)(n_parts * stride) + 255) / 256 * 256;
    const size_t part_bytes = (sizeof(F) * (size_t)((int64_t)n_parts * nblk * stride) + 255) / 256 * 256;
    const size_t csum_bytes = ((want_csum ? sizeof(F) * (size_t)(nblk * m) : 0) + 255) / 256 * 256 + 256;
    void *wsv = nullptr;
    int rc = get_workspace(tmp_bytes + part_bytes + csum_bytes + 256, &wsv, st);
    if (rc) return rc;
    F *tmp = reinterpret_cast<F *>(wsv);
    F *ws = reinterpret_cast<F *>(reinterpret_cast<char *>(wsv) + tmp_bytes);
    F *ws_csum = reinterpret_cast<F *>(reinterpret_cast<char *>(wsv) + tmp_bytes + part_bytes);
    const size_t lds = (size_t)EnLds<F>::TOTAL;
    auto kern = want_csum ? &csr_dense_ent_kernel<F, true> : &csr_dense_ent_kernel<F, false>;
    TM_HIP(hipFuncSetAttribute(reinterpret_cast<const void *>(kern),
                               hipFuncAttributeMaxDynamicSharedMemorySize, (int)lds));
    prof_begin(st);
    hipLaunchKernelGGL(kern, dim3((unsigned)nblk, (unsigned)n_parts, (unsigned)nz), dim3(EN_THREADS), lds, st,
                       vals, meta, bstart, n_groups, n_slabs, spb, B, n, r, (int)nB, d, ws, ws_csum,
                       reinterpret_cast<long long *>((uintptr_t)tune("ent_prof", 0)));
    prof_end(st);
    TM_LAUNCH_CHECK();
    rc = launch_reduce_partials<F>(ws, stride, (int)nblk, n_parts, tmp, n_parts * stride, false, st);
    if (rc) return rc;
    hipLaunchKernelGGL((en_untile_kernel<F>), dim3((unsigned)ceil_div(total, 256)), dim3(256), 0, st, tmp, m,
                       nB, out);
    TM_LAUNCH_CHECK();
    if (want_csum) {
        hipLaunchKernelGGL((en_csum_kernel<F>), dim3((unsigned)ceil_div(m, 256)), dim3(256), 0, st, ws_csum,
                           (int)nblk, m, colsum);
        TM_LAUNCH_CHECK();
    }
    return TM_OK;
}

}

extern "C" {
int tm_ent_rows(void) { return tmh::EN_R; }
int tm_ent_group_cols(void) { return tmh::EN_C; }
int tm_ent_batch_slots(void) { return tmh::EN_B; }

int tm_csr_dense_sandwich_ent_f32(const float *vals, const uint16_t *meta, const uint32_t *bstart, int64_t n,
                                  int64_t m, const float *B, int64_t r, const float *d, float *out,
                                  float *colsum, void *stream) {
    return tmh::run_csr_dense_ent<float>(vals, meta, bstart, n, m, B, r, d, out, colsum, tmh::as_stream(stream));
}
int tm_csr_dense_sandwich_ent_f64(const double *vals, const uint16_t *meta, const uint32_t *bstart, int64_t n,
                                  int64_t m, const double *B, int64_t r, const double *d, double *out,
                                  double *colsum, void *stream) {
    return tmh::run_csr_dense_ent<double>(vals, meta, bstart, n, m, B, r, d, out, colsum, tmh::as_stream(stream));
}
}
```

### tabmat_amd/csrc/syrk_co.hip

```cpp
#include <algorithm>

#include "common.hpp"

namespace tmh {

constexpr int CO_RS = 12;
constexpr int CO_W = 128;
constexpr int CO_LDW = CO_W + 16;
constexpr int CO_CPI = 64;
constexpr int CO_ITEM_ROWS = CO_CPI * CO_RS;
constexpr int CO_T = 36;
constexpr int CO_NWAVES = 4;
constexpr int CO_THREADS = CO_NWAVES * 64;
constexpr int CO_CHUNK = CO_RS * CO_LDW;
constexpr size_t CO_LDS = sizeof(double) * (size_t)(2 * CO_CHUNK + 2 * CO_RS) + 32 + sizeof(double) * CO_W;
constexpr size_t CO_LDS_TV = CO_LDS + sizeof(double) * 2 * CO_RS;

typedef double co_acc_t __attribute__((ext_vector_type(4)));
typedef double co_vec2 __attribute__((ext_vector_type(2)));

constexpr int co_tri_row(int t) {
    int r = 0;
    while ((r + 1) * (r + 2) / 2 <= t) ++r;
    return r;
}

__host__ __device__ constexpr int co_actual_col(int v) {
    return 32 * ((v >> 4) >> 1) + 2 * (v & 15) + ((v >> 4) & 1);
}

template <int WID, int S>
__device__ __forceinline__ void co_mfma_set(const double (&xa)[8], const double (&xb)[8],
                                            co_acc_t (&acc)[9]) {
    if constexpr (S < 9) {
        constexpr int t = WID + S * CO_NWAVES;
        constexpr int bi = co_tri_row(t);
        constexpr int bj = t - bi * (bi + 1) / 2;
        acc[S] = __builtin_amdgcn_mfma_f64_16x16x4f64(xa[bi], xb[bj], acc[S], 0, 0, 0);
        co_mfma_set<WID, S + 1>(xa, xb, acc);
    }
}

template <bool CEN, bool ODD, bool TV = false>
__global__ __launch_bounds__(CO_THREADS) __attribute__((amdgpu_waves_per_eu(TV ? 2 : 3)))
void syrk_co_kernel(const double *__restrict__ X, int64_t n, int64_t m, int n_cols,
                    const double *__restrict__ d, int n_items, unsigned *__restrict__ counter,
                    double *__restrict__ part, double *__restrict__ cpart, WgLogBuf *__restrict__ log,
                    const unsigned *__restrict__ only_if, const double *__restrict__ center,
                    const double *__restrict__ v = nullptr, double *__restrict__ vpart = nullptr) {
    if (only_if != nullptr && *only_if == 0) return;
    extern __shared__ __attribute__((aligned(16))) unsigned char smem_raw[];
    double *lds = reinterpret_cast<double *>(smem_raw);
    double *dl = lds + 2 * CO_CHUNK;
    unsigned *slot = reinterpret_cast<unsigned *>(dl + 2 * CO_RS);
    double *vl = reinterpret_cast<double *>(slot + 4) + CO_W;

    const int tid = threadIdx.x;
    const int lane = tid & 63;
    const int wave = __builtin_amdgcn_readfirstlane(tid >> 6);
    const unsigned long long t_begin = wg_log_begin(log);

    co_acc_t acc[9];
#pragma unroll
    for (int s = 0; s < 9; ++s) acc[s] = co_acc_t{0, 0, 0, 0};
    double cs0 = 0.0, cs1 = 0.0;
    double cv0 = 0.0, cv1 = 0.0;

    co_vec2 stage[3];
    double dstage = 0.0, vstage = 0.0;
    double *cl = reinterpret_cast<double *>(slot + 4);
    if constexpr (CEN) {
        if (tid < CO_W) cl[tid] = tid < n_cols ? center[tid] : 0.0;
    }

    unsigned idL = blockIdx.x;
    int oL = 0;
    unsigned idNext;
    if (tid == 0) *slot = gridDim.x + atomicAdd(counter, 1u);
    __syncthreads();
    idNext = *slot;
    bool pending = false;

    auto load_chunk = [&]() -> unsigned {
        const unsigned id = idL;
        const int64_t tb = (int64_t)id * CO_ITEM_ROWS + (int64_t)oL * CO_RS;
        if (tid < CO_RS) {
            const int64_t t = tb + tid;
            dstage = t < n ? d[t] : 0.0;
            if constexpr (TV) vstage = t < n ? v[t] : 0.0;
        }
#pragma unroll
        for (int i = 0; i < 3; ++i) {
            const int q = tid + i * CO_THREADS;
            const int r = q >> 6, c = (q & 63) * 2;
            const int64_t t = tb + r;
            co_vec2 v = co_vec2{0.0, 0.0};
            if (ODD && t + 1 >= n && c + 1 >= n_cols) {
                if (t < n && c < n_cols) v[0] = X[t * m + c];
            } else if (t < n && c < n_cols) {
                v = __builtin_nontemporal_load(reinterpret_cast<const co_vec2 *>(X + t * m + c));
            }
            stage[i] = v;
        }
        if (++oL == CO_CPI) {
            oL = 0;
            idL = idNext;
            if (tid == 0) *slot = gridDim.x + atomicAdd(counter, 1u);
            pending = true;
        }
        return id;
    };
    auto store_chunk = [&](int buf) {
        double *lb = lds + buf * CO_CHUNK;
        if (tid < CO_RS) dl[buf * CO_RS + tid] = dstage;
        if constexpr (TV) {
            if (tid < CO_RS) vl[buf * CO_RS + tid] = vstage;
        }
        co_vec2 cen = co_vec2{0.0, 0.0};
        if constexpr (CEN) cen = *reinterpret_cast<const co_vec2 *>(cl + (tid & 63) * 2);
#pragma unroll
        for (int i = 0; i < 3; ++i) {
            const int q = tid + i * CO_THREADS;
            *reinterpret_cast<co_vec2 *>(lb + (q >> 6) * CO_LDW + (q & 63) * 2) = CEN ? stage[i] - cen : stage[i];
        }
    };

    auto read_frag = [&](const double *lb, const double *db, int g, double (&xb)[8], double &dv, double &vv) {
        const int rl = 4 * g + (lane >> 4);
        dv = db[rl];
        if constexpr (TV) vv = db[rl + (vl - dl)];
        const double *lrow = lb + rl * CO_LDW + 2 * (lane & 15);
#pragma unroll
        for (int q = 0; q < 4; ++q) {
            const co_vec2 v = *reinterpret_cast<const co_vec2 *>(lrow + 32 * q);
            xb[2 * q] = v[0];
            xb[2 * q + 1] = v[1];
        }
    };

    auto run = [&](auto wid) {
        constexpr int WID = decltype(wid)::value;
        unsigned id_c = load_chunk();
        store_chunk(0);
        unsigned id_c1 = load_chunk();
        __syncthreads();
        if (pending) { idNext = *slot; pending = false; }
        int buf = 0;
        while (id_c < (unsigned)n_items) {
            const double *lb = lds + buf * CO_CHUNK;
            const double *db = dl + buf * CO_RS;
            double xb0[8], xb1[8], xa[8], dv0, dv1, vv0 = 0.0, vv1 = 0.0;
            read_frag(lb, db, 0, xb0, dv0, vv0);
            read_frag(lb, db, 1, xb1, dv1, vv1);
#pragma unroll
            for (int b = 0; b < 8; ++b) xa[b] = dv0 * xb0[b];
            cs0 += xa[2 * WID];
            cs1 += xa[2 * WID + 1];
            if constexpr (TV) {
                cv0 = __builtin_fma(vv0, xb0[2 * WID], cv0);
                cv1 = __builtin_fma(vv0, xb0[2 * WID + 1], cv1);
            }
            co_mfma_set<WID, 0>(xa, xb0, acc);
            store_chunk(buf ^ 1);
            const unsigned id_c2 = load_chunk();
            read_frag(lb, db, 2, xb0, dv0, vv0);
#pragma unroll
            for (int b = 0; b < 8; ++b) xa[b] = dv1 * xb1[b];
            cs0 += xa[2 * WID];
            cs1 += xa[2 * WID + 1];
            if constexpr (TV) {
                cv0 = __builtin_fma(vv1, xb1[2 * WID], cv0);
                cv1 = __builtin_fma(vv1, xb1[2 * WID + 1], cv1);
            }
            co_mfma_set<WID, 0>(xa, xb1, acc);
#pragma unroll
            for (int b = 0; b < 8; ++b) xa[b] = dv0 * xb0[b];
            cs0 += xa[2 * WID];
            cs1 += xa[2 * WID + 1];
            if constexpr (TV) {
                cv0 = __builtin_fma(vv0, xb0[2 * WID], cv0);
                cv1 = __builtin_fma(vv0, xb0[2 * WID + 1], cv1);
            }
            co_mfma_set<WID, 0>(xa, xb0, acc);
            __syncthreads();
            if (pending) { idNext = *slot; pending = false; }
            id_c = id_c1;
            id_c1 = id_c2;
            buf ^= 1;
        }
        double *dst = part + (int64_t)blockIdx.x * (CO_T * 256);
#pragma unroll
        for (int s = 0; s < 9; ++s) {
            const int t = WID + s * CO_NWAVES;
#pragma unroll
            for (int r = 0; r < 4; ++r)
                dst[t * 256 + ((lane >> 4) + 4 * r) * 16 + (lane & 15)] = acc[s][r];
        }
        cs0 += __shfl_xor(cs0, 16, 64);
        cs0 += __shfl_xor(cs0, 32, 64);
        cs1 += __shfl_xor(cs1, 16, 64);
        cs1 += __shfl_xor(cs1, 32, 64);
        if (lane < 16) {
            double *cd = cpart + (int64_t)blockIdx.x * CO_W;
            cd[32 * WID + 2 * lane] = cs0;
            cd[32 * WID + 2 * lane + 1] = cs1;
        }
        if constexpr (TV) {
            cv0 += __shfl_xor(cv0, 16, 64);
            cv0 += __shfl_xor(cv0, 32, 64);
            cv1 += __shfl_xor(cv1, 16, 64);
            cv1 += __shfl_xor(cv1, 32, 64);
            if (lane < 16) {
                double *vd = vpart + (int64_t)blockIdx.x * CO_W;
                vd[32 * WID + 2 * lane] = cv0;
                vd[32 * WID + 2 * lane + 1] = cv1;
            }
        }
    };
    if (wave == 0) run(std::integral_constant<int, 0>{});
    else if (wave == 1) run(std::integral_constant<int, 1>{});
    else if (wave == 2) run(std::integral_constant<int, 2>{});
    else run(std::integral_constant<int, 3>{});
    if (tid == 0) wg_log_end(log, t_begin, WG_SYRK_CO);
}

__global__ __launch_bounds__(1024) void syrk_co_finish_kernel(const double *__restrict__ part,
                                                              int nblk, int n_cols,
                                                              double *__restrict__ out, int64_t ldo,
                                                              const unsigned *__restrict__ only_if) {
    if (only_if != nullptr && *only_if == 0) return;
    __shared__ double red[16][64];
    const int e = blockIdx.y * 64 + threadIdx.x, s = threadIdx.y, t = blockIdx.x;
    double a = 0.0;
    for (int b = s; b < nblk; b += 16) a += part[((int64_t)b * CO_T + t) * 256 + e];
    red[s][threadIdx.x] = a;
    __syncthreads();
    if (s == 0) {
        double v = 0.0;
#pragma unroll
        for (int w = 0; w < 16; w += 4)
            v += (red[w][threadIdx.x] + red[w + 1][threadIdx.x]) +
                 (red[w + 2][threadIdx.x] + red[w + 3][threadIdx.x]);
        int bi = 0;
        while ((bi + 1) * (bi + 2) / 2 <= t) ++bi;
        const int bj = t - bi * (bi + 1) / 2;
        const int ci = co_actual_col(16 * bi + (e >> 4)), cj = co_actual_col(16 * bj + (e & 15));
        if (ci < n_cols && cj < n_cols && (bi != bj || (e >> 4) >= (e & 15))) {
            out[(int64_t)ci * ldo + cj] = v;
            if (ci != cj) out[(int64_t)cj * ldo + ci] = v;
        }
    }
}

__global__ __launch_bounds__(CO_W) void syrk_co_colsum_kernel(const double *__restrict__ cpart,
                                                              int nblk, int n_cols,
                                                              double *__restrict__ colsum,
                                                              const unsigned *__restrict__ only_if) {
    if (only_if != nullptr && *only_if == 0u) return;
    const int c = threadIdx.x;
    double a = 0.0;
    for (int b = 0; b < nblk; ++b) a += cpart[(int64_t)b * CO_W + c];
    if (c < n_cols) colsum[c] = a;
}

size_t syrk_co_ws_bytes() {
    const size_t grid = (size_t)std::max<int64_t>(1, tune("co_grid", 3 * NUM_CU));
    return 256 + sizeof(double) * grid * (CO_T * 256 + 2 * CO_W);
}

static int run_syrk_co_impl(const double *X, int64_t ldx, int64_t n, int64_t m, const double *d, double *out,
                            int64_t ldo, double *colsum, const unsigned *only_if, void *ws_given,
                            hipStream_t st, const double *center, const double *v, double *xtv) {
    TM_REQUIRE((v == nullptr) == (xtv == nullptr), "v and xtv go together");
    TM_REQUIRE(n >= 0 && m >= 0, "negative shape");
    TM_REQUIRE(m == 0 || syrk_co_ok(X, m),
               "the co-resident syrk takes a 16-byte aligned C-ordered block of <= 128 columns");
    if (m == 0) return TM_OK;
    if (n == 0) {
        TM_HIP(hipMemset2DAsync(out, sizeof(double) * (size_t)ldo, 0, sizeof(double) * (size_t)m, (size_t)m, st));
        if (colsum) TM_HIP(hipMemsetAsync(colsum, 0, sizeof(double) * (size_t)m, st));
        if (xtv) TM_HIP(hipMemsetAsync(xtv, 0, sizeof(double) * (size_t)m, st));
        return TM_OK;
    }
    const int64_t n_items64 = ceil_div(n, CO_ITEM_ROWS);
    TM_REQUIRE(n_items64 < (1ll << 31), "too many rows");
    const int n_items = (int)n_items64;
    const int grid = (int)std::min<int64_t>(n_items, tune("co_grid", 3 * NUM_CU));
    const size_t part_bytes = sizeof(double) * (size_t)grid * CO_T * 256;
    const size_t cpart_bytes = sizeof(double) * (size_t)grid * CO_W * (v ? 2 : 1);
    void *wsv = ws_given;
    if (wsv == nullptr) {
        int rc = get_workspace(256 + part_bytes + cpart_bytes, &wsv, st);
        if (rc) return rc;
    }
    unsigned *counter = reinterpret_cast<unsigned *>(wsv);
    double *part = reinterpret_cast<double *>(reinterpret_cast<char *>(wsv) + 256);
    double *cpart = part + (size_t)grid * CO_T * 256;
    double *vpart = v ? cpart + (size_t)grid * CO_W : nullptr;
    TM_HIP(hipMemsetAsync(counter, 0, 256, st));
    auto kern = v ? ((m & 1) ? (center ? &syrk_co_kernel<true, true, true> : &syrk_co_kernel<false, true, true>)
                             : (center ? &syrk_co_kernel<true, false, true> : &syrk_co_kernel<false, false, true>))
                  : ((m & 1) ? (center ? &syrk_co_kernel<true, true> : &syrk_co_kernel<false, true>)
                             : (center ? &syrk_co_kernel<true, false> : &syrk_co_kernel<false, false>));
    const size_t lds = v ? CO_LDS_TV : CO_LDS;
    TM_HIP(hipFuncSetAttribute(reinterpret_cast<const void *>(kern),
                               hipFuncAttributeMaxDynamicSharedMemorySize, (int)lds));
    prof_begin(st);
    hipLaunchKernelGGL(kern, dim3((unsigned)grid), dim3(CO_THREADS), lds, st, X, n, ldx,
                       (int)m, d, n_items, counter, part, cpart, wg_log_ptr(), only_if, center, v, vpart);
    prof_end(st);
    TM_LAUNCH_CHECK();
    hipLaunchKernelGGL(syrk_co_finish_kernel, dim3(CO_T, 4), dim3(64, 16), 0, st, part, grid, (int)m,
                       out, ldo, only_if);
    TM_LAUNCH_CHECK();
    if (colsum) {
        hipLaunchKernelGGL(syrk_co_colsum_kernel, dim3(1), dim3(CO_W), 0, st, cpart, grid, (int)m,
                           colsum, only_if);
        TM_LAUNCH_CHECK();
    }
    if (xtv) {
        hipLaunchKernelGGL(syrk_co_colsum_kernel, dim3(1), dim3(CO_W), 0, st, vpart, grid, (int)m,
                           xtv, only_if);
        TM_LAUNCH_CHECK();
    }
    return TM_OK;
}

int run_syrk_co(const double *X, int64_t n, int64_t m, const double *d, double *out, double *colsum,
                hipStream_t st, const double *center, const double *v, double *xtv) {
    return run_syrk_co_impl(X, m, n, m, d, out, m, colsum, nullptr, nullptr, st, center, v, xtv);
}

int run_syrk_co_flagged(const double *X, int64_t ldx, int64_t n, int64_t m, const double *d, double *out,
                        int64_t ldo, double *colsum, const unsigned *flag, void *ws, hipStream_t st,
                        const double *center, const double *v, double *xtv) {
    return run_syrk_co_impl(X, ldx, n, m, d, out, ldo, colsum, flag, ws, st, center, v, xtv);
}

}

using namespace tmh;

extern "C" {

int tm_dense_sandwich_co_f64(const double *X, int64_t n, int64_t m, const double *d, double *out,
                             double *colsum, void *stream) {
    return run_syrk_co(X, n, m, d, out, colsum, as_stream(stream));
}

int tm_dense_sandwich_co_centered_f64(const double *X, int64_t n, int64_t m, const double *d, const double *center,
                                      double *out, double *colsum, void *stream) {
    return run_syrk_co(X, n, m, d, out, colsum, as_stream(stream), center);
}

int tm_dense_sandwich_co_xtv_f64(const double *X, int64_t n, int64_t m, const double *d, const double *v,
                                 double *out, double *colsum, double *xtv, void *stream) {
    TM_REQUIRE(v != nullptr && xtv != nullptr, "v and xtv are required");
    return run_syrk_co(X, n, m, d, out, colsum, as_stream(stream), nullptr, v, xtv);
}

int tm_dense_sandwich_co_centered_xtv_f64(const double *X, int64_t n, int64_t m, const double *d, const double *v,
                                          const double *center, double *out, double *colsum, double *xtv,
                                          void *stream) {
    TM_REQUIRE(v != nullptr && xtv != nullptr, "v and xtv are required");
    return run_syrk_co(X, n, m, d, out, colsum, as_stream(stream), center, v, xtv);
}

}
```

### tabmat_amd/csrc/syrk_i8.hip

```cpp
#include <algorithm>
#include <cmath>

#include "common.hpp"

#if defined(I8_NO_SB)
#define I8_SB
#else
#define I8_SB __builtin_amdgcn_sched_barrier(0)
#endif
#if defined(I8_TRACE)
#define I8_STAMP(k)                                                                                     \
    do {                                                                                                \
        if (blockIdx.x == 0 && lane == 0 && trace_it >= 8 && trace_it < 12)                             \
            trace_buf[((trace_it - 8) * 4 + wave) * 8 + (k)] = __builtin_readcyclecounter();            \
    } while (0)
#else
#define I8_STAMP(k)
#endif
namespace tmh {

constexpr int I8_W = 128;
constexpr int I8_T = 36;
constexpr int I8_ND = 5;
constexpr int I8_WLO = 2;
constexpr int I8_NC = 2 * (I8_ND - 1) - I8_WLO + 1;
constexpr int I8_FBITS = 38;
constexpr int I8_RS = 64;
constexpr int I8_HS = 32;
constexpr int I8_WAVES = 4;
constexpr int I8_THREADS = I8_WAVES * 64;
constexpr int I8_PSTR = 64;
constexpr int I8_PLANE = I8_W * I8_PSTR;
constexpr int I8_PLANES = I8_ND * I8_PLANE;
constexpr int I8_RAWSTR = 1024 + 32;
constexpr int I8_RAWBUF = I8_HS * I8_RAWSTR;
#ifndef I8_DMA_AUX
#define I8_DMA_AUX 0
#endif
#ifndef I8_CPI_N
#define I8_CPI_N 32
#endif
constexpr int I8_CPI = I8_CPI_N;
constexpr int I8_ITEM_ROWS = I8_CPI * I8_RS;
constexpr size_t I8_LDS = (size_t)I8_PLANES + 3 * (size_t)I8_RAWBUF + 3 * I8_HS * sizeof(double) + 16;
static_assert(I8_LDS <= 160 * 1024, "planes + the ring of 3 half chunks fill the CU's LDS");

typedef int i8_v4 __attribute__((ext_vector_type(4)));

struct I8Info {
    unsigned dmax_bits_hi;
    unsigned dmax_bits_lo;
    unsigned flag;
    unsigned pad;
};

constexpr int i8_pair_find(int idx, bool want_s) {
    int k = 0;
    for (int w = I8_WLO; w <= 2 * (I8_ND - 1); ++w)
        for (int s = 0; s < I8_ND; ++s) {
            const int t = w - s;
            if (t < 0 || t >= I8_ND) continue;
            if (k == idx) return want_s ? s : t;
            ++k;
        }
    return -1;
}
constexpr int i8_pair_s(int idx) { return i8_pair_find(idx, true); }
constexpr int i8_pair_t(int idx) { return i8_pair_find(idx, false); }
constexpr int i8_count_pairs() {
    int k = 0;
    while (i8_pair_find(k, true) >= 0) ++k;
    return k;
}
constexpr int I8_NP = i8_count_pairs();
static_assert(I8_NP == 22, "the pair groups of the chunk loop are laid out for 22 pairs");

template <int WID>
struct I8Tiles {
    static constexpr int NB = 5;
    static constexpr int block(int l) {
        constexpr int B[4][5] = {{0, 1, 2, 3, 4}, {0, 1, 5, 6, 7}, {2, 3, 5, 6, 7}, {3, 4, 5, 6, 7}};
        return B[WID][l];
    }
    static constexpr int local(int b) {
        for (int l = 0; l < NB; ++l)
            if (block(l) == b) return l;
        return 0;
    }
    static constexpr int bi(int q) {
        constexpr int T[4][9] = {{1, 2, 3, 4, 2, 3, 4, 3, 4}, {5, 6, 7, 5, 6, 7, 6, 0, 1},
                                 {5, 6, 7, 5, 6, 7, 7, 2, 3}, {5, 6, 7, 4, 7, 4, 5, 6, 7}};
        return T[WID][q];
    }
    static constexpr int bj(int q) {
        constexpr int T[4][9] = {{0, 0, 0, 0, 1, 1, 1, 2, 2}, {0, 0, 0, 1, 1, 1, 5, 0, 1},
                                 {2, 2, 2, 3, 3, 3, 5, 2, 3}, {4, 4, 4, 3, 6, 4, 5, 6, 7}};
        return T[WID][q];
    }
    static constexpr int tile(int q) { return bi(q) * (bi(q) + 1) / 2 + bj(q); }
};

#if defined(__HIP_DEVICE_COMPILE__)
typedef __amdgpu_buffer_rsrc_t i8_rsrc_t;
__device__ __forceinline__ i8_rsrc_t i8_rsrc(const void *base, int64_t bytes) {
    const unsigned nb = bytes <= 0 ? 0u : (bytes > 0xFFFFFFFFll ? 0xFFFFFFFFu : (unsigned)bytes);
    return __builtin_amdgcn_make_buffer_rsrc(const_cast<void *>(base), 0, (int)nb, 0x00020000);
}
__device__ __forceinline__ void i8_dma16(i8_rsrc_t rs, void *lds, int voff) {
    __builtin_amdgcn_raw_ptr_buffer_load_lds(rs, (__attribute__((address_space(3))) void *)lds, 16, voff, 0, 0, I8_DMA_AUX);
}
__device__ __forceinline__ void i8_lds_barrier() { asm volatile("s_waitcnt lgkmcnt(0)\n\ts_barrier" ::: "memory"); }
__device__ __forceinline__ unsigned i8_perm(unsigned hi, unsigned lo, unsigned sel) {
    return __builtin_amdgcn_perm(hi, lo, sel);
}
#else
struct i8_rsrc_t {};
inline i8_rsrc_t i8_rsrc(const void *, int64_t) { return {}; }
inline void i8_dma16(i8_rsrc_t, void *, int) {}
inline void i8_lds_barrier() {}
inline unsigned i8_perm(unsigned, unsigned, unsigned) { return 0; }
#endif

__global__ __launch_bounds__(256) void i8_screen_kernel(const double *__restrict__ d, int64_t n, I8Info *info) {
    double mx = 0.0;
    bool bad = false;
    const int64_t stride = (int64_t)gridDim.x * blockDim.x;
    int64_t i = (int64_t)blockIdx.x * blockDim.x + threadIdx.x;
    for (; i + 3 * stride < n; i += 4 * stride) {
        const double v0 = d[i], v1 = d[i + stride], v2 = d[i + 2 * stride], v3 = d[i + 3 * stride];
        bad |= !(v0 >= 0.0) || !(v0 <= 1.7e308) || !(v1 >= 0.0) || !(v1 <= 1.7e308) ||
               !(v2 >= 0.0) || !(v2 <= 1.7e308) || !(v3 >= 0.0) || !(v3 <= 1.7e308);
        mx = fmax(fmax(mx, fmax(v0, v1)), fmax(v2, v3));
    }
    for (; i < n; i += stride) {
        const double v = d[i];
        bad |= !(v >= 0.0) || !(v <= 1.7e308);
        mx = fmax(mx, v);
    }
    for (int off = 32; off > 0; off >>= 1) {
        mx = fmax(mx, __shfl_down(mx, off, 64));
        bad |= (bool)__shfl_down((int)bad, off, 64);
    }
    __shared__ double wmx[4];
    __shared__ int wbad[4];
    if ((threadIdx.x & 63) == 0) {
        wmx[threadIdx.x >> 6] = mx;
        wbad[threadIdx.x >> 6] = (int)bad;
    }
    __syncthreads();
    if (threadIdx.x == 0) {
        mx = fmax(fmax(wmx[0], wmx[1]), fmax(wmx[2], wmx[3]));
        if (wbad[0] | wbad[1] | wbad[2] | wbad[3]) atomicOr(&info->flag, 1u);
        atomicMax(reinterpret_cast<unsigned long long *>(info), (unsigned long long)__double_as_longlong(mx > 0.0 ? mx : 0.0));
    }
}

__global__ void i8_scale_kernel(const double *__restrict__ colmax, int m, int64_t n_rows, I8Info *info,
                                double *__restrict__ sigma, double *__restrict__ rscale, int *history) {
    const int i = threadIdx.x;
    if (history != nullptr && i == 0) {
        const int calls = history[1]++;
        if (history[0] >= 3 && (calls & 31) != 0) atomicOr(&info->flag, 4u);
    }
    if (i >= I8_W) return;
    const double dmax = __longlong_as_double(*reinterpret_cast<const long long *>(info));
    if (history != nullptr && i < m && n_rows > 0) {
        const double prev = reinterpret_cast<const double *>(history + 4)[i];
        const double bound = fmin(64.0, 134217728.0 / (double)n_rows);
        if (prev > 0.0 && !(colmax[i] * colmax[i] * dmax <= bound * prev)) atomicOr(&info->flag, 4u);
    }
    __syncthreads();
    double s = 1.0, r = 1.0;
    if (i < m) {
        const double big = colmax[i] * sqrt(dmax);
        if (big > 0.0 && info->flag == 0) {
            int e;
            frexp(big, &e);
            s = ldexp(1.0, I8_FBITS - e);
            r = ldexp(1.0, e - I8_FBITS);
        }
    }
    sigma[i] = s;
    rscale[i] = r;
}

template <bool CSUM, bool CEN, bool TV = false>
__global__ __launch_bounds__(I8_THREADS) __attribute__((amdgpu_waves_per_eu(1, 1)))
void syrk_i8_kernel(const double *__restrict__ X, int64_t ldx, int64_t n, int64_t m, const double *__restrict__ d,
                    const double *__restrict__ sigma, const I8Info *__restrict__ info, int n_items,
                    unsigned *__restrict__ counter, double *__restrict__ part, double *__restrict__ colsum,
                    const double *__restrict__ center, const double *__restrict__ v = nullptr,
                    double *__restrict__ xtv = nullptr) {
    if (info->flag != 0) return;
    __shared__ __attribute__((aligned(16))) unsigned char planes[I8_PLANES];
    __shared__ __attribute__((aligned(16))) unsigned char raw[3 * I8_RAWBUF];
    __shared__ double dl[3 * I8_HS];
    __shared__ double vl[TV ? 3 * I8_HS : 1];
    __shared__ unsigned slot_mem[4];
    unsigned *slot = slot_mem;
#if defined(I8_TRACE)
    unsigned long long *trace_buf = reinterpret_cast<unsigned long long *>(reinterpret_cast<char *>(counter) - 256 + 2560);
    int trace_it = 0;
#endif

    const int tid = threadIdx.x;
    const int lane = tid & 63;
    const int wave = __builtin_amdgcn_readfirstlane(tid >> 6);
    const int cl = lane & 15, rq = lane >> 4;

    unsigned idL = blockIdx.x;
    int hL = 0;
    unsigned idNext;
    if (tid == 0) *slot = gridDim.x + atomicAdd(counter, 1u);
    __syncthreads();
    idNext = __builtin_amdgcn_readfirstlane(*slot);
    bool pending = false;

    using C0 = std::integral_constant<int, 0>;
    using C1 = std::integral_constant<int, 1>;
    double dreg = 0.0, vreg = 0.0;
    const int dma_voff = lane * 2 < m ? lane * 16 : 0x7ffffff0;
    auto issue_half = [&](int rb) -> unsigned {
        const unsigned id = idL;
        const int64_t tb = (int64_t)id * I8_ITEM_ROWS + (int64_t)hL * I8_HS;
        const int64_t left = min((n - tb) * ldx * 8, (int64_t)I8_HS * ldx * 8);
        const uint64_t xb = (uint64_t)(uintptr_t)(X + tb * ldx);
        const unsigned xlo = __builtin_amdgcn_readfirstlane((unsigned)xb);
        const unsigned xhi = __builtin_amdgcn_readfirstlane((unsigned)(xb >> 32));
        const unsigned nbytes = __builtin_amdgcn_readfirstlane(
            left <= 0 ? 0u : (left > 0xFFFFFFFFll ? 0xFFFFFFFFu : (unsigned)left));
        const i8_rsrc_t rs = i8_rsrc(reinterpret_cast<const void *>((uintptr_t)(((uint64_t)xhi << 32) | xlo)), nbytes);
        if (wave == 0 && lane < I8_HS) dreg = tb + lane < n ? d[tb + lane] : 0.0;
        if constexpr (TV) {
            if (wave == 0 && lane < I8_HS) vreg = tb + lane < n ? v[tb + lane] : 0.0;
        }
#if !defined(I8_ABLATE_NO_DMA)
#pragma unroll
        for (int j = 0; j < 8; ++j)
            i8_dma16(rs, raw + rb * I8_RAWBUF + (8 * wave + j) * I8_RAWSTR, (int)((8 * wave + j) * ldx * 8) + dma_voff);
#endif
        if (++hL == 2 * I8_CPI) {
            hL = 0;
            idL = idNext;
            if (tid == 0) *slot = gridDim.x + atomicAdd(counter, 1u);
            pending = true;
        }
        return id;
    };
    auto publish_d = [&](int rb) {
        if (wave == 0 && lane < I8_HS) dl[rb * I8_HS + lane] = sqrt(dreg);
        if constexpr (TV) {
            if (wave == 0 && lane < I8_HS) vl[rb * I8_HS + lane] = vreg;
        }
    };

    const double sg0 = sigma[32 * wave + cl], sg1 = sigma[32 * wave + 16 + cl];
    double cen0 = 0.0, cen1 = 0.0;
    if constexpr (CEN) {
        cen0 = 32 * wave + cl < m ? center[32 * wave + cl] : 0.0;
        cen1 = 32 * wave + 16 + cl < m ? center[32 * wave + 16 + cl] : 0.0;
    }
    double cs0 = 0.0, cs1 = 0.0;
    double cv0 = 0.0, cv1 = 0.0;
    const double MAGIC = 6755399441055744.0 + 551911719040.0;
    const unsigned raw_lds = (unsigned)(uintptr_t)(__attribute__((address_space(3))) unsigned char *)raw;
    const unsigned planes_lds = (unsigned)(uintptr_t)(__attribute__((address_space(3))) unsigned char *)planes;
    struct Quad { double x[4]; };
    auto quad_issue = [&](int rb, auto cb_c, auto qq_c) -> Quad {
        constexpr int cb = decltype(cb_c)::value, qq = decltype(qq_c)::value;
        Quad q;
#if defined(I8_ABLATE_NO_CONVERT) || defined(I8_ABLATE_DMA_ONLY)
        q.x[0] = q.x[1] = q.x[2] = q.x[3] = 0.0;
        return q;
#endif
        const int col = 32 * wave + 16 * cb + cl;
        const int row0 = 4 * (rq + 4 * qq);
        const unsigned ra = raw_lds + (unsigned)(rb * I8_RAWBUF + row0 * I8_RAWSTR + col * 8);
#if defined(__HIP_DEVICE_COMPILE__)
        asm volatile("ds_read_b64 %0, %4\n\tds_read_b64 %1, %4 offset:1056\n\tds_read_b64 %2, %4 offset:2112\n\t"
                     "ds_read_b64 %3, %4 offset:3168"
                     : "=&v"(q.x[0]), "=&v"(q.x[1]), "=&v"(q.x[2]), "=&v"(q.x[3])
                     : "v"(ra)
                     : "memory");
#else
        (void)ra;
        q.x[0] = q.x[1] = q.x[2] = q.x[3] = 0.0;
#endif
        static_assert(I8_RAWSTR == 1056, "the ds_read offsets above are multiples of the raw row stride");
        return q;
    };
    auto quad_wait = [&](Quad &q) {
#if defined(__HIP_DEVICE_COMPILE__) && !defined(I8_ABLATE_NO_CONVERT) && !defined(I8_ABLATE_DMA_ONLY)
        asm volatile("s_waitcnt lgkmcnt(0)" : "+v"(q.x[0]), "+v"(q.x[1]), "+v"(q.x[2]), "+v"(q.x[3])::"memory");
#endif
    };
    struct Conv {
        double dv[4];
        double vv[TV ? 4 : 1];
        unsigned lo[4], hi[4];
        unsigned t[4], h[2], g[5];
    };
    auto conv_step = [&](auto k_c, const Quad &q, Conv &c, int rb, int hh, auto cb_c, auto qq_c) {
        constexpr int k = decltype(k_c)::value;
        constexpr int cb = decltype(cb_c)::value, qq = decltype(qq_c)::value;
#if defined(I8_ABLATE_NO_CONVERT) || defined(I8_ABLATE_DMA_ONLY)
        return;
#endif
        const int row0 = 4 * (rq + 4 * qq);
        if constexpr (k == 0) {
#pragma unroll
            for (int j = 0; j < 4; ++j) c.dv[j] = dl[rb * I8_HS + row0 + j];
            if constexpr (TV) {
#pragma unroll
                for (int j = 0; j < 4; ++j) c.vv[j] = vl[rb * I8_HS + row0 + j];
            }
        } else if constexpr (k >= 1 && k <= 4) {
            const double sg = cb ? sg1 : sg0;
            double xv = q.x[k - 1];
            if constexpr (CEN) xv -= cb ? cen1 : cen0;
            const double u = xv * c.dv[k - 1];
            const double t = __builtin_fma(u, sg, MAGIC);
            if constexpr (CSUM) {
                if constexpr (cb) cs1 = __builtin_fma(u, c.dv[k - 1], cs1);
                else cs0 = __builtin_fma(u, c.dv[k - 1], cs0);
            }
            if constexpr (TV) {
                if constexpr (cb) cv1 = __builtin_fma(xv, c.vv[k - 1], cv1);
                else cv0 = __builtin_fma(xv, c.vv[k - 1], cv0);
            }
            c.lo[k - 1] = (unsigned)__double2loint(t);
            c.hi[k - 1] = (unsigned)__double2hiint(t);
        } else if constexpr (k == 5) {
            c.t[0] = i8_perm(c.lo[1], c.lo[0], 0x05010400u);
            c.t[1] = i8_perm(c.lo[1], c.lo[0], 0x07030602u);
        } else if constexpr (k == 6) {
            c.t[2] = i8_perm(c.lo[3], c.lo[2], 0x05010400u);
            c.t[3] = i8_perm(c.lo[3], c.lo[2], 0x07030602u);
        } else if constexpr (k == 7) {
            c.g[0] = i8_perm(c.t[2], c.t[0], 0x05040100u) ^ 0x80808080u;
        } else if constexpr (k == 8) {
            c.g[1] = i8_perm(c.t[2], c.t[0], 0x07060302u) ^ 0x80808080u;
        } else if constexpr (k == 9) {
            c.g[2] = i8_perm(c.t[3], c.t[1], 0x05040100u) ^ 0x80808080u;
        } else if constexpr (k == 10) {
            c.g[3] = i8_perm(c.t[3], c.t[1], 0x07060302u) ^ 0x80808080u;
        } else if constexpr (k == 11) {
            c.h[0] = i8_perm(c.hi[1], c.hi[0], 0x05010400u);
            c.h[1] = i8_perm(c.hi[3], c.hi[2], 0x05010400u);
        } else if constexpr (k == 12) {
            c.g[4] = i8_perm(c.h[1], c.h[0], 0x05040100u) ^ 0x80808080u;
        } else if constexpr (k == 13) {
            const int col = 32 * wave + 16 * cb + cl;
            const unsigned pa =
                planes_lds + (unsigned)(col * I8_PSTR + (((2 * hh + qq) ^ ((cl >> 1) & 3)) << 4) + 4 * rq);
#if defined(__HIP_DEVICE_COMPILE__)
            asm volatile("ds_write_b32 %0, %1\n\tds_write_b32 %0, %2 offset:8192\n\tds_write_b32 %0, %3 offset:16384\n\t"
                         "ds_write_b32 %0, %4 offset:24576\n\tds_write_b32 %0, %5 offset:32768"
                         :
                         : "v"(pa), "v"(c.g[0]), "v"(c.g[1]), "v"(c.g[2]), "v"(c.g[3]), "v"(c.g[4])
                         : "memory");
#else
            (void)pa;
#endif
            static_assert(I8_PLANE == 8192 && I8_ND == 5, "the ds_write offsets above are the plane strides");
        }
    };
    constexpr int I8_CSTEPS = 14;
    constexpr int I8_CLAT = 3;
    auto quad_convert = [&](const Quad &q, int rb, int hh, auto cb_c, auto qq_c) {
        Conv c;
        static_for<I8_CSTEPS>([&](auto kc) { conv_step(kc, q, c, rb, hh, cb_c, qq_c); });
    };
    auto convert_quad = [&](int rb, int hh, auto cb_c, auto qq_c) {
        Quad q = quad_issue(rb, cb_c, qq_c);
        quad_wait(q);
        quad_convert(q, rb, hh, cb_c, qq_c);
    };
    auto convert_half = [&](int rb, int hh) {
        convert_quad(rb, hh, C0{}, C0{});
        convert_quad(rb, hh, C0{}, C1{});
        convert_quad(rb, hh, C1{}, C0{});
        convert_quad(rb, hh, C1{}, C1{});
    };

    const int foff = (lane & 15) * I8_PSTR + (((lane >> 4) ^ ((lane >> 1) & 3)) << 4);
    auto frag = [&](int b, int s) {
        return *reinterpret_cast<const i8_v4 *>(planes + s * I8_PLANE + b * 16 * I8_PSTR + foff);
    };

    auto run = [&](auto wid) {
        constexpr int WID = decltype(wid)::value;
        i8_v4 acc[9][I8_NC];
        double *dst = part + (int64_t)blockIdx.x * (I8_T * 256);
        auto flush = [&]() {
            asm volatile("s_nop 15\n\ts_nop 7" ::: "memory");
            unsigned lane_off = (unsigned)(((4 * (lane >> 4)) * 16 + (lane & 15)) * 8);
            asm volatile("" : "+v"(lane_off));
            char *const fb = reinterpret_cast<char *>(dst) + lane_off;
            static_for<9>([&](auto sc) {
                constexpr int s9 = decltype(sc)::value;
                constexpr int t = I8Tiles<WID>::tile(s9);
#pragma unroll
                for (int r = 0; r < 4; ++r) {
                    double v = (double)acc[s9][I8_NC - 1][r];
#pragma unroll
                    for (int c = I8_NC - 2; c >= 0; --c) v = v * 256.0 + (double)acc[s9][c][r];
                    atomicAdd(reinterpret_cast<double *>(fb + (t * 256 + r * 16) * 8), v);
                }
            });
        };

        unsigned id_c = issue_half(0);
        asm volatile("s_waitcnt vmcnt(8)" ::: "memory");
        publish_d(0);
        (void)issue_half(1);
        asm volatile("s_waitcnt vmcnt(8)" ::: "memory");
        publish_d(1);
        asm volatile("s_waitcnt vmcnt(0)" ::: "memory");
        i8_lds_barrier();
        if (pending) { idNext = __builtin_amdgcn_readfirstlane(*slot); pending = false; }
        convert_half(0, 0);
        convert_half(1, 1);
        i8_lds_barrier();
        unsigned id_c1 = issue_half(2);
        asm volatile("s_waitcnt vmcnt(8)" ::: "memory");
        publish_d(2);
        (void)issue_half(0);
        asm volatile("s_waitcnt vmcnt(8)" ::: "memory");
        publish_d(0);
        int sa = 2;

        while (id_c < (unsigned)n_items) {
#pragma unroll
          for (int t = 0; t < 9; ++t)
#pragma unroll
              for (int c = 0; c < I8_NC; ++c) {
                  acc[t][c] = i8_v4{0, 0, 0, 0};
                  asm volatile("" : "+a"(acc[t][c]));
              }
          for (int oc = 0; oc < I8_CPI; ++oc) {
            I8_STAMP(0);
            const int sb = sa == 2 ? 0 : sa + 1;
            const int sc = sb == 2 ? 0 : sb + 1;
            i8_lds_barrier();
            I8_STAMP(1);
            if (pending) { idNext = __builtin_amdgcn_readfirstlane(*slot); pending = false; }
            Quad qa = quad_issue(sa, C0{}, C0{});
            using TL = I8Tiles<WID>;
            i8_v4 F[TL::NB][I8_ND];
            auto mf = [&](auto lo_c, auto hi_c) {
                constexpr int LO = decltype(lo_c)::value, HI = decltype(hi_c)::value;
                static_for<HI - LO>([&](auto ic) {
                    constexpr int k = LO + decltype(ic)::value;
                    constexpr int idx = k / 9, q = k % 9;
                    constexpr int ps = i8_pair_s(idx), pt = i8_pair_t(idx);
#if defined(I8_ABLATE_DMA_ONLY)
                    return;
#endif
                    i8_v4 &cacc = acc[q][ps + pt - I8_WLO];
                    const i8_v4 fa = F[TL::local(TL::bi(q))][ps], fb = F[TL::local(TL::bj(q))][pt];
                    asm volatile("v_mfma_i32_16x16x64_i8 %0, %1, %2, %0" : "+a"(cacc) : "v"(fa), "v"(fb));
                });
            };
#define I8_MF(lo, hi) mf(std::integral_constant<int, lo>{}, std::integral_constant<int, hi>{})
            static_for<I8_ND>([&](auto oc_) {
                constexpr int order[I8_ND] = {0, 2, 1, 3, 4};
                constexpr int sd = order[decltype(oc_)::value];
#pragma unroll
                for (int b = 0; b < TL::NB; ++b) {
#if defined(I8_ABLATE_DMA_ONLY)
                    F[b][sd] = i8_v4{0, 0, 0, 0};
#else
                    F[b][sd] = frag(TL::block(b), sd);
#endif
                }
            });
            static_assert(i8_pair_s(0) == 0 && i8_pair_t(0) == 2 && i8_pair_s(2) == 2 && i8_pair_s(3) + i8_pair_t(3) == 3,
                          "the first three pairs are class 2");
            I8_MF(0, 27);
#if !defined(I8_NO_WEAVE)
            __builtin_amdgcn_sched_group_barrier(0x100, 10, 0);
            static_for<15>([&](auto) {
                __builtin_amdgcn_sched_group_barrier(0x008, 1, 0);
                __builtin_amdgcn_sched_group_barrier(0x100, 1, 0);
            });
            __builtin_amdgcn_sched_group_barrier(0x008, 12, 0);
#endif
            I8_SB;
            I8_STAMP(2);
            i8_lds_barrier();
            I8_STAMP(3);
            quad_wait(qa);
            const unsigned id_a = issue_half(sc);
            auto group = [&](auto lo_c, auto hi_c, const Quad &q, int rb, int hh, auto cb_c, auto qq_c) {
                constexpr int LO = decltype(lo_c)::value, HI = decltype(hi_c)::value;
                static_assert(HI - LO >= I8_CSTEPS + I8_CLAT, "a group holds all steps of one quad");
                Conv c;
                static_for<HI - LO>([&](auto ic) {
                    constexpr int i = decltype(ic)::value;
                    mf(std::integral_constant<int, LO + i>{}, std::integral_constant<int, LO + i + 1>{});
                    if constexpr (i == 0) conv_step(std::integral_constant<int, 0>{}, q, c, rb, hh, cb_c, qq_c);
                    if constexpr (i > I8_CLAT && i - I8_CLAT < I8_CSTEPS)
                        conv_step(std::integral_constant<int, i - I8_CLAT>{}, q, c, rb, hh, cb_c, qq_c);
                    I8_SB;
                });
            };
#define I8_GROUP(lo, hi, q, rb, hh, cb, qq) \
    group(std::integral_constant<int, lo>{}, std::integral_constant<int, hi>{}, q, rb, hh, cb, qq)
            Quad qb = quad_issue(sa, C0{}, C1{});
            I8_GROUP(27, 49, qa, sa, 0, C0{}, C0{});
            quad_wait(qb);
            I8_SB;
            qa = quad_issue(sa, C1{}, C0{});
            I8_GROUP(49, 71, qb, sa, 0, C0{}, C1{});
            quad_wait(qa);
            I8_SB;
            qb = quad_issue(sa, C1{}, C1{});
            I8_GROUP(71, 93, qa, sa, 0, C1{}, C0{});
            quad_wait(qb);
            I8_SB;
            I8_GROUP(93, 114, qb, sa, 0, C1{}, C1{});
            I8_SB;
            I8_STAMP(4);
            asm volatile("s_waitcnt vmcnt(8)" ::: "memory");
            publish_d(sc);
            I8_STAMP(5);
            i8_lds_barrier();
            I8_STAMP(6);
            (void)issue_half(sa);
            qa = quad_issue(sb, C0{}, C0{});
            I8_MF(114, 120);
            quad_wait(qa);
            I8_SB;
            qb = quad_issue(sb, C0{}, C1{});
            I8_GROUP(120, 140, qa, sb, 1, C0{}, C0{});
            quad_wait(qb);
            I8_SB;
            qa = quad_issue(sb, C1{}, C0{});
            I8_GROUP(140, 160, qb, sb, 1, C0{}, C1{});
            quad_wait(qa);
            I8_SB;
            qb = quad_issue(sb, C1{}, C1{});
            I8_GROUP(160, 180, qa, sb, 1, C1{}, C0{});
            quad_wait(qb);
            I8_SB;
            I8_GROUP(180, 198, qb, sb, 1, C1{}, C1{});
            I8_SB;
#undef I8_MF
#undef I8_GROUP
            static_assert(I8_NP * 9 == 198, "the group bounds above");
            I8_STAMP(7);
            asm volatile("s_waitcnt vmcnt(8)" ::: "memory");
            publish_d(sa);
#if defined(I8_TRACE)
            ++trace_it;
#endif
            sa = sc;
            id_c = id_c1;
            id_c1 = id_a;
          }
          flush();
        }
    };
    if (wave == 0) run(std::integral_constant<int, 0>{});
    else if (wave == 1) run(std::integral_constant<int, 1>{});
    else if (wave == 2) run(std::integral_constant<int, 2>{});
    else run(std::integral_constant<int, 3>{});
    asm volatile("s_waitcnt vmcnt(0)" ::: "memory");
    if constexpr (CSUM) {
        cs0 += __shfl_xor(cs0, 16, 64);
        cs0 += __shfl_xor(cs0, 32, 64);
        cs1 += __shfl_xor(cs1, 16, 64);
        cs1 += __shfl_xor(cs1, 32, 64);
        if (lane < 16) {
            if (32 * wave + cl < m) atomicAdd(colsum + 32 * wave + cl, cs0);
            if (32 * wave + 16 + cl < m) atomicAdd(colsum + 32 * wave + 16 + cl, cs1);
        }
    }
    if constexpr (TV) {
        cv0 += __shfl_xor(cv0, 16, 64);
        cv0 += __shfl_xor(cv0, 32, 64);
        cv1 += __shfl_xor(cv1, 16, 64);
        cv1 += __shfl_xor(cv1, 32, 64);
        if (lane < 16) {
            if (32 * wave + cl < m) atomicAdd(xtv + 32 * wave + cl, cv0);
            if (32 * wave + 16 + cl < m) atomicAdd(xtv + 32 * wave + 16 + cl, cv1);
        }
    }
}

__global__ __launch_bounds__(1024) void syrk_i8_finish_kernel(const double *__restrict__ part, int nblk,
                                                              int n_cols, const double *__restrict__ rscale,
                                                              const I8Info *__restrict__ info,
                                                              double *__restrict__ out, int64_t ldo) {
    if (info->flag != 0) return;
#if defined(I8_TRACE)
    if (blockIdx.x == 0 && blockIdx.y == 0 && threadIdx.y == 0) {
        const unsigned long long *tb = reinterpret_cast<const unsigned long long *>(reinterpret_cast<const char *>(info) + 2560);
        for (int k = threadIdx.x; k < 128; k += 64) out[k] = (double)(tb[k] - tb[0]);
    }
    return;
#endif
    __shared__ double red[16][64];
    const int e = blockIdx.y * 64 + threadIdx.x, s = threadIdx.y, t = blockIdx.x;
    double a = 0.0;
    for (int b = s; b < nblk; b += 16) a += part[((int64_t)b * I8_T + t) * 256 + e];
    red[s][threadIdx.x] = a;
    __syncthreads();
    if (s == 0) {
        double v = 0.0;
#pragma unroll
        for (int w = 0; w < 16; w += 4)
            v += (red[w][threadIdx.x] + red[w + 1][threadIdx.x]) + (red[w + 2][threadIdx.x] + red[w + 3][threadIdx.x]);
        int bi = 0;
        while ((bi + 1) * (bi + 2) / 2 <= t) ++bi;
        const int bj = t - bi * (bi + 1) / 2;
        const int ci = 16 * bi + (e >> 4), cj = 16 * bj + (e & 15);
        if (ci < n_cols && cj < n_cols && (bi != bj || (e >> 4) >= (e & 15))) {
            v = v * 65536.0 * rscale[ci] * rscale[cj];
            static_assert(I8_WLO == 2, "65536 = 256^I8_WLO");
            out[(int64_t)ci * ldo + cj] = v;
            if (ci != cj) out[(int64_t)cj * ldo + ci] = v;
        }
    }
}

__global__ void i8_envelope_kernel(const double *__restrict__ out, int64_t ldo, const double *__restrict__ colmax,
                                   int m, int64_t n, I8Info *info, int *history) {
    const int j = threadIdx.x;
    __shared__ int miss;
    if (j == 0) miss = 0;
    __syncthreads();
    const bool live = info->flag == 0;
#if defined(I8_TRACE)
    return;
#endif
    if (j < m && live) {
        const double dmax = __longlong_as_double(*reinterpret_cast<const long long *>(info));
        const double big2 = colmax[j] * colmax[j] * dmax;
        const double bound = fmin(64.0, 134217728.0 / (double)n);
        if (!(big2 <= bound * out[(int64_t)j * ldo + j])) {
            atomicOr(&info->flag, 2u);
            miss = 1;
        }
    }
    __syncthreads();
    if (history != nullptr && j == 0 && live) history[0] = miss ? history[0] + 1 : 0;
}

__global__ void i8_record_diag_kernel(const double *__restrict__ out, int64_t ldo, int m, int *history) {
    const int j = threadIdx.x;
    if (j < I8_W) reinterpret_cast<double *>(history + 4)[j] = j < m ? out[(int64_t)j * ldo + j] : 0.0;
}

int run_syrk_co_flagged(const double *X, int64_t ldx, int64_t n, int64_t m, const double *d, double *out,
                        int64_t ldo, double *colsum, const unsigned *flag, void *ws, hipStream_t st,
                        const double *center, const double *v, double *xtv);
size_t syrk_co_ws_bytes();

int run_syrk_i8_panel(const double *X, int64_t ldx, int64_t n, int64_t m, const double *d, const double *colmax,
                      double *out, int64_t ldo, double *colsum, int *history, hipStream_t st, const double *center,
                      const double *v, double *xtv) {
    TM_REQUIRE((v == nullptr) == (xtv == nullptr), "v and xtv go together");
    TM_REQUIRE(v == nullptr || colsum == nullptr, "X' d and X' v are not built into one int8 kernel");
    TM_REQUIRE(n >= 0 && m >= 0, "negative shape");
    TM_REQUIRE(ldx >= m && ldo >= m, "row strides");
    TM_REQUIRE(m == 0 || syrk_co_ok(X, m), "the int8 syrk takes a 16-byte aligned C-ordered f64 block of <= 128 columns");
    if (m == 0) return TM_OK;
    if (n == 0) {
        TM_HIP(hipMemset2DAsync(out, sizeof(double) * (size_t)ldo, 0, sizeof(double) * (size_t)m, (size_t)m, st));
        if (colsum) TM_HIP(hipMemsetAsync(colsum, 0, sizeof(double) * (size_t)m, st));
        if (xtv) TM_HIP(hipMemsetAsync(xtv, 0, sizeof(double) * (size_t)m, st));
        return TM_OK;
    }
    if (colsum) TM_HIP(hipMemsetAsync(colsum, 0, sizeof(double) * (size_t)m, st));
    if (xtv) TM_HIP(hipMemsetAsync(xtv, 0, sizeof(double) * (size_t)m, st));
    const int64_t n_items64 = ceil_div(n, I8_ITEM_ROWS);
    TM_REQUIRE(n_items64 < (1ll << 31), "too many rows");
    const int n_items = (int)n_items64;
    const int grid = (int)std::max<int64_t>(1, std::min<int64_t>(n_items, tune("i8_grid", NUM_CU)));
    const size_t part_bytes = sizeof(double) * (size_t)grid * I8_T * 256;
    const size_t own_bytes = (4096 + part_bytes + 255) / 256 * 256;
    void *wsv = nullptr;
    int rc = get_workspace(own_bytes + syrk_co_ws_bytes(), &wsv, st);
    if (rc) return rc;
    char *wb = reinterpret_cast<char *>(wsv);
    I8Info *info = reinterpret_cast<I8Info *>(wb);
    unsigned *counter = reinterpret_cast<unsigned *>(wb + 256);
    double *sigma = reinterpret_cast<double *>(wb + 512);
    double *rscale = reinterpret_cast<double *>(wb + 512 + 1024);
    double *part = reinterpret_cast<double *>(wb + 4096);
    TM_HIP(hipMemsetAsync(wb, 0, 4096 + part_bytes, st));
    const int sgrid = (int)std::min<int64_t>(4 * NUM_CU, ceil_div(n, 1024));
    hipLaunchKernelGGL(i8_screen_kernel, dim3((unsigned)sgrid), dim3(256), 0, st, d, n, info);
    hipLaunchKernelGGL(i8_scale_kernel, dim3(1), dim3(I8_W), 0, st, colmax, (int)m, n, info, sigma, rscale, history);
    TM_LAUNCH_CHECK();
    prof_begin(st);
    auto go = [&](auto kern) {
        hipLaunchKernelGGL(kern, dim3((unsigned)grid), dim3(I8_THREADS), 0, st, X, ldx, n, m, d, sigma, info, n_items,
                           counter, part, colsum, center, v, xtv);
    };
    if (v) {
        if (center) go(syrk_i8_kernel<false, true, true>);
        else go(syrk_i8_kernel<false, false, true>);
    } else if (center) {
        if (colsum) go(syrk_i8_kernel<true, true>);
        else go(syrk_i8_kernel<false, true>);
    } else {
        if (colsum) go(syrk_i8_kernel<true, false>);
        else go(syrk_i8_kernel<false, false>);
    }
    prof_end(st);
    TM_LAUNCH_CHECK();
    hipLaunchKernelGGL(syrk_i8_finish_kernel, dim3(I8_T, 4), dim3(64, 16), 0, st, part, grid, (int)m, rscale, info,
                       out, ldo);
    hipLaunchKernelGGL(i8_envelope_kernel, dim3(1), dim3(I8_W), 0, st, out, ldo, colmax, (int)m, n, info, history);
    TM_LAUNCH_CHECK();
    prof_hold(true);
    rc = run_syrk_co_flagged(X, ldx, n, m, d, out, ldo, colsum, &info->flag, wb + own_bytes, st, center, v, xtv);
    prof_hold(false);
    if (rc == TM_OK && history != nullptr) {
        hipLaunchKernelGGL(i8_record_diag_kernel, dim3(1), dim3(I8_W), 0, st, out, ldo, (int)m, history);
        TM_LAUNCH_CHECK();
    }
    return rc;
}

int run_syrk_i8(const double *X, int64_t n, int64_t m, const double *d, const double *colmax, double *out,
                double *colsum, int *history, hipStream_t st, const double *center = nullptr,
                const double *v = nullptr, double *xtv = nullptr) {
    return run_syrk_i8_panel(X, m, n, m, d, colmax, out, m, colsum, history, st, center, v, xtv);
}

}

extern "C" {

int tm_dense_sandwich_i8_history_words(void) { return 4 + 2 * tmh::I8_W; }

int tm_dense_sandwich_i8_f64(const double *X, int64_t n, int64_t m, const double *d, const double *colmax,
                             double *out, void *stream) {
    return tmh::run_syrk_i8(X, n, m, d, colmax, out, nullptr, nullptr, tmh::as_stream(stream));
}

int tm_dense_sandwich_i8_xtd_f64(const double *X, int64_t n, int64_t m, const double *d, const double *colmax,
                                 double *out, double *colsum, void *stream) {
    return tmh::run_syrk_i8(X, n, m, d, colmax, out, colsum, nullptr, tmh::as_stream(stream));
}

int tm_dense_sandwich_i8_hist_f64(const double *X, int64_t n, int64_t m, const double *d, const double *colmax,
                                  double *out, double *colsum, int32_t *history, void *stream) {
    return tmh::run_syrk_i8(X, n, m, d, colmax, out, colsum, history, tmh::as_stream(stream));
}

int tm_dense_sandwich_i8_centered_f64(const double *X, int64_t n, int64_t m, const double *d, const double *colmax,
                                      const double *center, double *out, double *colsum, int32_t *history,
                                      void *stream) {
    return tmh::run_syrk_i8(X, n, m, d, colmax, out, colsum, history, tmh::as_stream(stream), center);
}

int tm_dense_sandwich_i8_xtv_f64(const double *X, int64_t n, int64_t m, const double *d, const double *v,
                                 const double *colmax, double *out, double *xtv, int32_t *history, void *stream) {
    TM_REQUIRE(v != nullptr && xtv != nullptr, "v and xtv are required");
    return tmh::run_syrk_i8(X, n, m, d, colmax, out, nullptr, history, tmh::as_stream(stream), nullptr, v, xtv);
}

int tm_dense_sandwich_i8_centered_xtv_f64(const double *X, int64_t n, int64_t m, const double *d, const double *v,
                                          const double *colmax, const double *center, double *out, double *xtv,
                                          int32_t *history, void *stream) {
    TM_REQUIRE(v != nullptr && xtv != nullptr, "v and xtv are required");
    return tmh::run_syrk_i8(X, n, m, d, colmax, out, nullptr, history, tmh::as_stream(stream), center, v, xtv);
}

}
```

Baseline: 1072 GB/s.

## Fuse partial reductions with untile/assemble stores and merge int8 syrk helper kernels

Adds a map-based reduce kernel that writes the reduced partials directly into the final layout. This replaces the separate untile and assemble kernels and their temporary buffers for the categorical, sparse-blocks and CSR-dense paths, and it skips partial slots that no workgroup wrote, so the memset of the sparse-blocks workspace is dropped. In the int8 syrk path, the screen and scale kernels are merged through a last-arrival ticket, the envelope check and diagonal recording are folded into the finish kernels, and a large memset shrinks. Together this cuts kernel launches and extra HBM round trips, at the cost of more complex cross-block synchronisation and scattered output writes.

```diff
diff --git a/tabmat_amd/csrc/cat_multi.hip b/tabmat_amd/csrc/cat_multi.hip
--- a/tabmat_amd/csrc/cat_multi.hip
+++ b/tabmat_amd/csrc/cat_multi.hip
@@ -236,14 +236,15 @@
     store_tile(tile, cs.total, TJ, TJ, workgroup_slice(ws, stride));
 }
 
-template <typename F>
-__global__ void multi_cat_untile_kernel(const F *__restrict__ tmp, int64_t total, int64_t m,
-                                        int TJ, F *__restrict__ out) {
-    const int64_t e = (int64_t)blockIdx.x * blockDim.x + threadIdx.x;
-    if (e >= total * m) return;
-    const int64_t a = e / m, j = e % m;
-    out[e] = tmp[((j / TJ) * total + a) * TJ + (j % TJ)];
-}
+struct MultiCatUntileMap : ReduceMapAllLive {
+    int64_t m;
+    int TJ;
+    template <typename F>
+    __device__ void store(F *__restrict__ out, int part, int64_t e, F v) const {
+        const int64_t a = e / TJ, j = (int64_t)part * TJ + (e % TJ);
+        if (j < m) out[a * m + j] = v;
+    }
+};
 
 template <typename F, bool STAGE>
 __global__ __launch_bounds__(1024) void multi_cat_sparse_kernel(
@@ -773,12 +774,10 @@
 static int launch_and_finish(Kern kern, int64_t nblk, int64_t parts, int threads, size_t lds, const CatSet &cs,
                              int part_cols, int64_t m, F *out, hipStream_t st, Launch &&launch) {
     const int64_t stride = (int64_t)cs.total * part_cols;
-    const size_t tmp_bytes = ((sizeof(F) * (size_t)(parts * stride) + 255) / 256) * 256;
     void *wsv = nullptr;
-    int rc = get_workspace(tmp_bytes + sizeof(F) * (size_t)(parts * nblk * stride) + 256, &wsv, st);
+    int rc = get_workspace(sizeof(F) * (size_t)(parts * nblk * stride) + 256, &wsv, st);
     if (rc) return rc;
-    F *tmp = reinterpret_cast<F *>(wsv);
-    F *ws = reinterpret_cast<F *>(reinterpret_cast<char *>(wsv) + tmp_bytes);
+    F *ws = reinterpret_cast<F *>(wsv);
     if (lds > 48 * 1024)
         TM_HIP(hipFuncSetAttribute(reinterpret_cast<const void *>(kern), hipFuncAttributeMaxDynamicSharedMemorySize,
                                    (int)lds));
@@ -786,12 +785,10 @@
     launch(dim3((unsigned)nblk, (unsigned)parts), dim3((unsigned)threads), ws, stride);
     prof_end(st);
     TM_LAUNCH_CHECK();
-    rc = launch_reduce_partials<F>(ws, stride, (int)nblk, (int)parts, tmp, parts * stride, false, st);
-    if (rc) return rc;
-    hipLaunchKernelGGL((multi_cat_untile_kernel<F>), dim3((unsigned)ceil_div((int64_t)cs.total * m, 256)), dim3(256), 0,
-                       st, tmp, (int64_t)cs.total, m, part_cols, out);
-    TM_LAUNCH_CHECK();
-    return TM_OK;
+    MultiCatUntileMap untile;
+    untile.m = m;
+    untile.TJ = part_cols;
+    return launch_reduce_partials_map<F>(ws, stride, (int)nblk, (int)parts, out, untile, st);
 }
 
 template <int MAX_NC, int OVER = MAX_NC, int NC = 1, typename Fn>
diff --git a/tabmat_amd/csrc/reduce.hpp b/tabmat_amd/csrc/reduce.hpp
--- a/tabmat_amd/csrc/reduce.hpp
+++ b/tabmat_amd/csrc/reduce.hpp
@@ -58,6 +58,54 @@
     return TM_OK;
 }
 
+template <typename F, int NW, typename Map>
+__global__ __launch_bounds__(NW * 64) void reduce_partials_map_kernel(const F *__restrict__ ws, int64_t stride,
+                                                                      int nb, F *__restrict__ out, Map map) {
+    __shared__ double red[NW][64];
+    extern __shared__ __attribute__((aligned(16))) unsigned char map_lds[];
+    const int lane = threadIdx.x & 63;
+    const int wave = threadIdx.x >> 6;
+    const int64_t e = (int64_t)blockIdx.x * 64 + lane;
+    const int part = blockIdx.y;
+    map.begin(part, map_lds);
+    double acc = 0.0;
+    if (e < stride) {
+        const F *p = ws + ((int64_t)part * nb) * stride + e;
+        for (int b = wave; b < nb; b += NW)
+            if (map.live(map_lds, b)) acc += (double)p[(int64_t)b * stride];
+    }
+    red[wave][lane] = acc;
+    __syncthreads();
+    if (wave == 0 && e < stride) {
+        double s = 0.0;
+#pragma unroll
+        for (int w = 0; w < NW; w += 4)
+            s += (red[w][lane] + red[w + 1][lane]) + (red[w + 2][lane] + red[w + 3][lane]);
+        map.store(out, part, e, (F)s);
+    }
+}
+
+struct ReduceMapAllLive {
+    size_t lds_bytes() const { return 0; }
+    __device__ void begin(int, unsigned char *) const {}
+    __device__ bool live(const unsigned char *, int) const { return true; }
+};
+
+template <typename F, typename Map>
+inline int launch_reduce_partials_map(const F *ws, int64_t stride, int nb, int n_parts, F *out, const Map &map,
+                                      hipStream_t st) {
+    dim3 grid((unsigned)ceil_div(stride, 64), (unsigned)n_parts);
+    const bool small = (int64_t)grid.x * grid.y < 1024 && nb > 16;
+    if (small)
+        hipLaunchKernelGGL((reduce_partials_map_kernel<F, 16, Map>), grid, dim3(1024), map.lds_bytes(), st, ws,
+                           stride, nb, out, map);
+    else
+        hipLaunchKernelGGL((reduce_partials_map_kernel<F, 4, Map>), grid, dim3(256), map.lds_bytes(), st, ws, stride,
+                           nb, out, map);
+    TM_LAUNCH_CHECK();
+    return TM_OK;
+}
+
 __global__ void fill_i32_kernel(int32_t *p, int64_t n, int32_t v);
 __global__ void scatter_iota_i32_kernel(int32_t *map, const int32_t *cols, int64_t n_cols);
 
diff --git a/tabmat_amd/csrc/sparse_blocks.hip b/tabmat_amd/csrc/sparse_blocks.hip
--- a/tabmat_amd/csrc/sparse_blocks.hip
+++ b/tabmat_amd/csrc/sparse_blocks.hip
@@ -8,16 +8,42 @@
 constexpr int KB_WAVES = 16;
 constexpr int KB_TS = 128;
 
-template <typename F>
-__global__ void blocks_assemble_kernel(const F *__restrict__ tiles, int n_out, F *__restrict__ out) {
-    const int j = blockIdx.x * blockDim.x + threadIdx.x;
-    const int i = blockIdx.y;
-    if (i >= n_out || j >= n_out) return;
-    const int hi = max(i, j), lo = min(i, j);
-    const int I = hi / KB_TS, J = lo / KB_TS;
-    const int part = I * (I + 1) / 2 + J;
-    out[(int64_t)i * n_out + j] = tiles[(int64_t)part * KB_TS * KB_TS + (hi % KB_TS) * KB_TS + (lo % KB_TS)];
-}
+__device__ __forceinline__ void kb_tile_of_part(int part, int *I_out, int *J_out) {
+    int I = (int)((sqrtf(8.0f * (float)part + 1.0f) - 1.0f) * 0.5f);
+    while ((I + 1) * (I + 2) / 2 <= part) ++I;
+    while (I * (I + 1) / 2 > part) --I;
+    *I_out = I;
+    *J_out = part - I * (I + 1) / 2;
+}
+
+struct BlocksFinishMap {
+    const int4 *wg_tab;
+    int n_wg, max_nb, n_out;
+    size_t lds_bytes() const { return sizeof(unsigned) * (size_t)ceil_div(max_nb, 32); }
+    __device__ void begin(int part, unsigned char *lds) const {
+        unsigned *mask = reinterpret_cast<unsigned *>(lds);
+        for (int k = threadIdx.x; k < (max_nb + 31) / 32; k += blockDim.x) mask[k] = 0u;
+        __syncthreads();
+        for (int g = threadIdx.x; g < n_wg; g += blockDim.x) {
+            const int2 ps = *reinterpret_cast<const int2 *>(wg_tab + 2 * g);
+            if (ps.x == part && ps.y >= 0 && ps.y < max_nb) atomicOr(&mask[ps.y >> 5], 1u << (ps.y & 31));
+        }
+        __syncthreads();
+    }
+    __device__ bool live(const unsigned char *lds, int b) const {
+        return (reinterpret_cast<const unsigned *>(lds)[b >> 5] >> (b & 31)) & 1u;
+    }
+    template <typename F>
+    __device__ void store(F *__restrict__ out, int part, int64_t e, F v) const {
+        int I, J;
+        kb_tile_of_part(part, &I, &J);
+        const int r = (int)(e / KB_TS), c = (int)(e % KB_TS);
+        const int hi = I * KB_TS + r, lo = J * KB_TS + c;
+        if (hi >= n_out || lo > hi) return;
+        out[(int64_t)hi * n_out + lo] = v;
+        if (lo != hi) out[(int64_t)lo * n_out + hi] = v;
+    }
+};
 
 constexpr int KB_FLAG_REP_A = 1 << 16;
 constexpr int KB_FLAG_REP_B = 1 << 17;
@@ -215,14 +241,17 @@
     TM_REQUIRE(!D12 || n < (1ll << 24), "12-byte block descriptors hold 24 bits of row");
     TM_REQUIRE(max_nb >= 1 && n_wg >= 1, "empty workgroup table");
     const size_t lds = sizeof(lds_acc_t) * (size_t)(TS * TS);
-    const size_t tmp_bytes = (sizeof(F) * (size_t)n_parts * TS * TS + 255) / 256 * 256;
     const size_t ws_bytes = sizeof(F) * (size_t)n_parts * (size_t)max_nb * TS * TS;
+    BlocksFinishMap finish;
+    finish.wg_tab = reinterpret_cast<const int4 *>(wg_tab);
+    finish.n_wg = n_wg;
+    finish.max_nb = max_nb;
+    finish.n_out = (int)m;
+    TM_REQUIRE(finish.lds_bytes() <= 32 * 1024, "too many partial slots per tile");
     void *wsv = nullptr;
-    int rc = get_workspace(tmp_bytes + ws_bytes + 256, &wsv, st);
+    int rc = get_workspace(ws_bytes + 256, &wsv, st);
     if (rc) return rc;
-    F *tmp = reinterpret_cast<F *>(wsv);
-    F *ws = reinterpret_cast<F *>(reinterpret_cast<char *>(wsv) + tmp_bytes);
-    TM_HIP(hipMemsetAsync(ws, 0, ws_bytes, st));
+    F *ws = reinterpret_cast<F *>(wsv);
     auto kern = &sparse_sandwich_blocks_kernel<F, U8, D12>;
     TM_HIP(hipFuncSetAttribute(reinterpret_cast<const void *>(kern),
                                hipFuncAttributeMaxDynamicSharedMemorySize, (int)lds));
@@ -233,13 +262,7 @@
                        max_nb, ws, wg_log_ptr());
     prof_end(st);
     TM_LAUNCH_CHECK();
-    rc = launch_reduce_partials<F>(ws, (int64_t)TS * TS, max_nb, n_parts, tmp, (int64_t)n_parts * TS * TS,
-                                   false, st);
-    if (rc) return rc;
-    hipLaunchKernelGGL((blocks_assemble_kernel<F>), dim3((unsigned)ceil_div(m, 64), (unsigned)m), dim3(64),
-                       0, st, tmp, (int)m, out);
-    TM_LAUNCH_CHECK();
-    return TM_OK;
+    return launch_reduce_partials_map<F>(ws, (int64_t)TS * TS, max_nb, n_parts, out, finish, st);
 }
 
 }
diff --git a/tabmat_amd/csrc/sparse_ent.hip b/tabmat_amd/csrc/sparse_ent.hip
--- a/tabmat_amd/csrc/sparse_ent.hip
+++ b/tabmat_amd/csrc/sparse_ent.hip
@@ -341,13 +341,14 @@
     }
 }
 
-template <typename F>
-__global__ void en_untile_kernel(const F *__restrict__ tmp, int64_t m, int64_t nB, F *__restrict__ out) {
-    const int64_t e = (int64_t)blockIdx.x * blockDim.x + threadIdx.x;
-    if (e >= m * nB) return;
-    const int64_t i = e / nB, j = e % nB;
-    out[e] = tmp[((j / EN_W) * m + i) * EN_W + (j % EN_W)];
-}
+struct EnUntileMap : ReduceMapAllLive {
+    int64_t nB;
+    template <typename F>
+    __device__ void store(F *__restrict__ out, int part, int64_t e, F v) const {
+        const int64_t i = e / EN_W, j = (int64_t)part * EN_W + (e % EN_W);
+        if (j < nB) out[i * nB + j] = v;
+    }
+};
 
 template <typename F>
 __global__ void en_csum_kernel(const F *__restrict__ part, int nblk, int64_t m, F *__restrict__ csum) {
@@ -392,15 +393,13 @@
     const int64_t spb = ceil_div(n_slabs, nblk);
     nblk = ceil_div(n_slabs, spb);
     const int64_t stride = m * EN_W;
-    const size_t tmp_bytes = (sizeof(F) * (size_t)(n_parts * stride) + 255) / 256 * 256;
     const size_t part_bytes = (sizeof(F) * (size_t)((int64_t)n_parts * nblk * stride) + 255) / 256 * 256;
     const size_t csum_bytes = ((want_csum ? sizeof(F) * (size_t)(nblk * m) : 0) + 255) / 256 * 256 + 256;
     void *wsv = nullptr;
-    int rc = get_workspace(tmp_bytes + part_bytes + csum_bytes + 256, &wsv, st);
+    int rc = get_workspace(part_bytes + csum_bytes + 256, &wsv, st);
     if (rc) return rc;
-    F *tmp = reinterpret_cast<F *>(wsv);
-    F *ws = reinterpret_cast<F *>(reinterpret_cast<char *>(wsv) + tmp_bytes);
-    F *ws_csum = reinterpret_cast<F *>(reinterpret_cast<char *>(wsv) + tmp_bytes + part_bytes);
+    F *ws = reinterpret_cast<F *>(wsv);
+    F *ws_csum = reinterpret_cast<F *>(reinterpret_cast<char *>(wsv) + part_bytes);
     const size_t lds = (size_t)EnLds<F>::TOTAL;
     auto kern = want_csum ? &csr_dense_ent_kernel<F, true> : &csr_dense_ent_kernel<F, false>;
     TM_HIP(hipFuncSetAttribute(reinterpret_cast<const void *>(kern),
@@ -411,11 +410,10 @@
                        reinterpret_cast<long long *>((uintptr_t)tune("ent_prof", 0)));
     prof_end(st);
     TM_LAUNCH_CHECK();
-    rc = launch_reduce_partials<F>(ws, stride, (int)nblk, n_parts, tmp, n_parts * stride, false, st);
+    EnUntileMap untile;
+    untile.nB = nB;
+    rc = launch_reduce_partials_map<F>(ws, stride, (int)nblk, n_parts, out, untile, st);
     if (rc) return rc;
-    hipLaunchKernelGGL((en_untile_kernel<F>), dim3((unsigned)ceil_div(total, 256)), dim3(256), 0, st, tmp, m,
-                       nB, out);
-    TM_LAUNCH_CHECK();
     if (want_csum) {
         hipLaunchKernelGGL((en_csum_kernel<F>), dim3((unsigned)ceil_div(m, 256)), dim3(256), 0, st, ws_csum,
                            (int)nblk, m, colsum);
diff --git a/tabmat_amd/csrc/syrk_co.hip b/tabmat_amd/csrc/syrk_co.hip
--- a/tabmat_amd/csrc/syrk_co.hip
+++ b/tabmat_amd/csrc/syrk_co.hip
@@ -227,7 +227,8 @@
 __global__ __launch_bounds__(1024) void syrk_co_finish_kernel(const double *__restrict__ part,
                                                               int nblk, int n_cols,
                                                               double *__restrict__ out, int64_t ldo,
-                                                              const unsigned *__restrict__ only_if) {
+                                                              const unsigned *__restrict__ only_if,
+                                                              double *__restrict__ diag) {
     if (only_if != nullptr && *only_if == 0) return;
     __shared__ double red[16][64];
     const int e = blockIdx.y * 64 + threadIdx.x, s = threadIdx.y, t = blockIdx.x;
@@ -248,7 +249,10 @@
         if (ci < n_cols && cj < n_cols && (bi != bj || (e >> 4) >= (e & 15))) {
             out[(int64_t)ci * ldo + cj] = v;
             if (ci != cj) out[(int64_t)cj * ldo + ci] = v;
-        }
+            else if (diag != nullptr) diag[ci] = v;
+        }
+        if (diag != nullptr && t == 0 && blockIdx.y == 0)
+            for (int j = n_cols + (int)threadIdx.x; j < CO_W; j += 64) diag[j] = 0.0;
     }
 }
 
@@ -270,7 +274,8 @@
 
 static int run_syrk_co_impl(const double *X, int64_t ldx, int64_t n, int64_t m, const double *d, double *out,
                             int64_t ldo, double *colsum, const unsigned *only_if, void *ws_given,
-                            hipStream_t st, const double *center, const double *v, double *xtv) {
+                            hipStream_t st, const double *center, const double *v, double *xtv,
+                            double *diag = nullptr, bool counter_cleared = false) {
     TM_REQUIRE((v == nullptr) == (xtv == nullptr), "v and xtv go together");
     TM_REQUIRE(n >= 0 && m >= 0, "negative shape");
     TM_REQUIRE(m == 0 || syrk_co_ok(X, m),
@@ -297,7 +302,7 @@
     double *part = reinterpret_cast<double *>(reinterpret_cast<char *>(wsv) + 256);
     double *cpart = part + (size_t)grid * CO_T * 256;
     double *vpart = v ? cpart + (size_t)grid * CO_W : nullptr;
-    TM_HIP(hipMemsetAsync(counter, 0, 256, st));
+    if (!counter_cleared) TM_HIP(hipMemsetAsync(counter, 0, 256, st));
     auto kern = v ? ((m & 1) ? (center ? &syrk_co_kernel<true, true, true> : &syrk_co_kernel<false, true, true>)
                              : (center ? &syrk_co_kernel<true, false, true> : &syrk_co_kernel<false, false, true>))
                   : ((m & 1) ? (center ? &syrk_co_kernel<true, true> : &syrk_co_kernel<false, true>)
@@ -311,7 +316,7 @@
     prof_end(st);
     TM_LAUNCH_CHECK();
     hipLaunchKernelGGL(syrk_co_finish_kernel, dim3(CO_T, 4), dim3(64, 16), 0, st, part, grid, (int)m,
-                       out, ldo, only_if);
+                       out, ldo, only_if, diag);
     TM_LAUNCH_CHECK();
     if (colsum) {
         hipLaunchKernelGGL(syrk_co_colsum_kernel, dim3(1), dim3(CO_W), 0, st, cpart, grid, (int)m,
@@ -333,8 +338,8 @@
 
 int run_syrk_co_flagged(const double *X, int64_t ldx, int64_t n, int64_t m, const double *d, double *out,
                         int64_t ldo, double *colsum, const unsigned *flag, void *ws, hipStream_t st,
-                        const double *center, const double *v, double *xtv) {
-    return run_syrk_co_impl(X, ldx, n, m, d, out, ldo, colsum, flag, ws, st, center, v, xtv);
+                        const double *center, const double *v, double *xtv, double *diag) {
+    return run_syrk_co_impl(X, ldx, n, m, d, out, ldo, colsum, flag, ws, st, center, v, xtv, diag, true);
 }
 
 }
diff --git a/tabmat_amd/csrc/syrk_i8.hip b/tabmat_amd/csrc/syrk_i8.hip
--- a/tabmat_amd/csrc/syrk_i8.hip
+++ b/tabmat_amd/csrc/syrk_i8.hip
@@ -121,11 +121,38 @@
 inline unsigned i8_perm(unsigned, unsigned, unsigned) { return 0; }
 #endif
 
-__global__ __launch_bounds__(256) void i8_screen_kernel(const double *__restrict__ d, int64_t n, I8Info *info) {
+__device__ __forceinline__ bool i8_last_arrival(unsigned *ticket, unsigned total) {
+    __builtin_amdgcn_fence(__ATOMIC_RELEASE, "agent");
+    asm volatile("s_waitcnt vmcnt(0)" ::: "memory");
+    const unsigned t = __hip_atomic_fetch_add(ticket, 1u, __ATOMIC_RELAXED, __HIP_MEMORY_SCOPE_AGENT);
+    if (t + 1u != total) return false;
+    __builtin_amdgcn_fence(__ATOMIC_ACQUIRE, "agent");
+    return true;
+}
+__device__ __forceinline__ unsigned i8_flag_now(const I8Info *info) {
+    return __hip_atomic_load(&info->flag, __ATOMIC_RELAXED, __HIP_MEMORY_SCOPE_AGENT);
+}
+__device__ __forceinline__ double i8_dmax_now(const I8Info *info) {
+    return __longlong_as_double((long long)__hip_atomic_load(reinterpret_cast<const unsigned long long *>(info),
+                                                             __ATOMIC_RELAXED, __HIP_MEMORY_SCOPE_AGENT));
+}
+
+__global__ __launch_bounds__(256) void i8_screen_kernel(const double *__restrict__ d, int64_t n, I8Info *info,
+                                                        unsigned *ticket, double *__restrict__ zero, int64_t n_zero2,
+                                                        unsigned *__restrict__ co_counter,
+                                                        const double *__restrict__ colmax, int m,
+                                                        double *__restrict__ sigma, double *__restrict__ rscale,
+                                                        int *history) {
+    const int64_t stride = (int64_t)gridDim.x * blockDim.x;
+    int64_t i = (int64_t)blockIdx.x * blockDim.x + threadIdx.x;
+    {
+        typedef double i8_d2 __attribute__((ext_vector_type(2)));
+        i8_d2 *z = reinterpret_cast<i8_d2 *>(zero);
+        for (int64_t k = i; k < n_zero2; k += stride) z[k] = i8_d2{0.0, 0.0};
+        if (blockIdx.x == 0 && threadIdx.x < 64) co_counter[threadIdx.x] = 0u;
+    }
     double mx = 0.0;
     bool bad = false;
-    const int64_t stride = (int64_t)gridDim.x * blockDim.x;
-    int64_t i = (int64_t)blockIdx.x * blockDim.x + threadIdx.x;
     for (; i + 3 * stride < n; i += 4 * stride) {
         const double v0 = d[i], v1 = d[i + stride], v2 = d[i + 2 * stride], v3 = d[i + 3 * stride];
         bad |= !(v0 >= 0.0) || !(v0 <= 1.7e308) || !(v1 >= 0.0) || !(v1 <= 1.7e308) ||
@@ -143,6 +170,7 @@
     }
     __shared__ double wmx[4];
     __shared__ int wbad[4];
+    __shared__ int last;
     if ((threadIdx.x & 63) == 0) {
         wmx[threadIdx.x >> 6] = mx;
         wbad[threadIdx.x >> 6] = (int)bad;
@@ -152,36 +180,38 @@
         mx = fmax(fmax(wmx[0], wmx[1]), fmax(wmx[2], wmx[3]));
         if (wbad[0] | wbad[1] | wbad[2] | wbad[3]) atomicOr(&info->flag, 1u);
         atomicMax(reinterpret_cast<unsigned long long *>(info), (unsigned long long)__double_as_longlong(mx > 0.0 ? mx : 0.0));
-    }
-}
-
-__global__ void i8_scale_kernel(const double *__restrict__ colmax, int m, int64_t n_rows, I8Info *info,
-                                double *__restrict__ sigma, double *__restrict__ rscale, int *history) {
-    const int i = threadIdx.x;
-    if (history != nullptr && i == 0) {
+        last = (int)i8_last_arrival(ticket, gridDim.x);
+    }
+    __syncthreads();
+    if (!last) return;
+
+    const int c = threadIdx.x;
+    if (history != nullptr && c == 0) {
         const int calls = history[1]++;
         if (history[0] >= 3 && (calls & 31) != 0) atomicOr(&info->flag, 4u);
     }
-    if (i >= I8_W) return;
-    const double dmax = __longlong_as_double(*reinterpret_cast<const long long *>(info));
-    if (history != nullptr && i < m && n_rows > 0) {
-        const double prev = reinterpret_cast<const double *>(history + 4)[i];
-        const double bound = fmin(64.0, 134217728.0 / (double)n_rows);
-        if (prev > 0.0 && !(colmax[i] * colmax[i] * dmax <= bound * prev)) atomicOr(&info->flag, 4u);
-    }
+    const double dmax = i8_dmax_now(info);
+    if (history != nullptr && c < m && n > 0) {
+        const double prev = reinterpret_cast<const double *>(history + 4)[c];
+        const double bound = fmin(64.0, 134217728.0 / (double)n);
+        if (prev > 0.0 && !(colmax[c] * colmax[c] * dmax <= bound * prev)) atomicOr(&info->flag, 4u);
+    }
+    __builtin_amdgcn_fence(__ATOMIC_RELEASE, "agent");
+    asm volatile("s_waitcnt vmcnt(0)" ::: "memory");
     __syncthreads();
+    if (c >= I8_W) return;
     double s = 1.0, r = 1.0;
-    if (i < m) {
-        const double big = colmax[i] * sqrt(dmax);
-        if (big > 0.0 && info->flag == 0) {
+    if (c < m) {
+        const double big = colmax[c] * sqrt(dmax);
+        if (big > 0.0 && i8_flag_now(info) == 0) {
             int e;
             frexp(big, &e);
             s = ldexp(1.0, I8_FBITS - e);
             r = ldexp(1.0, e - I8_FBITS);
         }
     }
-    sigma[i] = s;
-    rscale[i] = r;
+    sigma[c] = s;
+    rscale[c] = r;
 }
 
 template <bool CSUM, bool CEN, bool TV = false>
@@ -591,9 +621,10 @@
 
 __global__ __launch_bounds__(1024) void syrk_i8_finish_kernel(const double *__restrict__ part, int nblk,
                                                               int n_cols, const double *__restrict__ rscale,
-                                                              const I8Info *__restrict__ info,
-                                                              double *__restrict__ out, int64_t ldo) {
-    if (info->flag != 0) return;
+                                                              I8Info *info, double *__restrict__ out, int64_t ldo,
+                                                              const double *__restrict__ colmax, int64_t n,
+                                                              int *history, unsigned *ticket) {
+    if ((i8_flag_now(info) & ~2u) != 0) return;
 #if defined(I8_TRACE)
     if (blockIdx.x == 0 && blockIdx.y == 0 && threadIdx.y == 0) {
         const unsigned long long *tb = reinterpret_cast<const unsigned long long *>(reinterpret_cast<const char *>(info) + 2560);
@@ -620,42 +651,26 @@
             v = v * 65536.0 * rscale[ci] * rscale[cj];
             static_assert(I8_WLO == 2, "65536 = 256^I8_WLO");
             out[(int64_t)ci * ldo + cj] = v;
-            if (ci != cj) out[(int64_t)cj * ldo + ci] = v;
-        }
-    }
-}
-
-__global__ void i8_envelope_kernel(const double *__restrict__ out, int64_t ldo, const double *__restrict__ colmax,
-                                   int m, int64_t n, I8Info *info, int *history) {
-    const int j = threadIdx.x;
-    __shared__ int miss;
-    if (j == 0) miss = 0;
-    __syncthreads();
-    const bool live = info->flag == 0;
-#if defined(I8_TRACE)
-    return;
-#endif
-    if (j < m && live) {
-        const double dmax = __longlong_as_double(*reinterpret_cast<const long long *>(info));
-        const double big2 = colmax[j] * colmax[j] * dmax;
-        const double bound = fmin(64.0, 134217728.0 / (double)n);
-        if (!(big2 <= bound * out[(int64_t)j * ldo + j])) {
-            atomicOr(&info->flag, 2u);
-            miss = 1;
-        }
-    }
-    __syncthreads();
-    if (history != nullptr && j == 0 && live) history[0] = miss ? history[0] + 1 : 0;
-}
-
-__global__ void i8_record_diag_kernel(const double *__restrict__ out, int64_t ldo, int m, int *history) {
-    const int j = threadIdx.x;
-    if (j < I8_W) reinterpret_cast<double *>(history + 4)[j] = j < m ? out[(int64_t)j * ldo + j] : 0.0;
+            if (ci != cj) {
+                out[(int64_t)cj * ldo + ci] = v;
+            } else {
+                const double big2 = colmax[ci] * colmax[ci] * i8_dmax_now(info);
+                const double bound = fmin(64.0, 134217728.0 / (double)n);
+                if (!(big2 <= bound * v)) atomicOr(&info->flag, 2u);
+                if (history != nullptr) reinterpret_cast<double *>(history + 4)[ci] = v;
+            }
+        }
+        if (history == nullptr) return;
+        if (t == 0 && blockIdx.y == 0)
+            for (int j = n_cols + (int)threadIdx.x; j < I8_W; j += 64) reinterpret_cast<double *>(history + 4)[j] = 0.0;
+        if (threadIdx.x == 0 && i8_last_arrival(ticket, gridDim.x * gridDim.y))
+            history[0] = (i8_flag_now(info) & 2u) ? history[0] + 1 : 0;
+    }
 }
 
 int run_syrk_co_flagged(const double *X, int64_t ldx, int64_t n, int64_t m, const double *d, double *out,
                         int64_t ldo, double *colsum, const unsigned *flag, void *ws, hipStream_t st,
-                        const double *center, const double *v, double *xtv);
+                        const double *center, const double *v, double *xtv, double *diag);
 size_t syrk_co_ws_bytes();
 
 int run_syrk_i8_panel(const double *X, int64_t ldx, int64_t n, int64_t m, const double *d, const double *colmax,
@@ -689,11 +704,14 @@
     unsigned *counter = reinterpret_cast<unsigned *>(wb + 256);
     double *sigma = reinterpret_cast<double *>(wb + 512);
     double *rscale = reinterpret_cast<double *>(wb + 512 + 1024);
+    unsigned *ticket_pre = reinterpret_cast<unsigned *>(wb + 64);
+    unsigned *ticket_fin = reinterpret_cast<unsigned *>(wb + 128);
     double *part = reinterpret_cast<double *>(wb + 4096);
-    TM_HIP(hipMemsetAsync(wb, 0, 4096 + part_bytes, st));
+    unsigned *co_counter = reinterpret_cast<unsigned *>(wb + own_bytes);
+    TM_HIP(hipMemsetAsync(wb, 0, 4096, st));
     const int sgrid = (int)std::min<int64_t>(4 * NUM_CU, ceil_div(n, 1024));
-    hipLaunchKernelGGL(i8_screen_kernel, dim3((unsigned)sgrid), dim3(256), 0, st, d, n, info);
-    hipLaunchKernelGGL(i8_scale_kernel, dim3(1), dim3(I8_W), 0, st, colmax, (int)m, n, info, sigma, rscale, history);
+    hipLaunchKernelGGL(i8_screen_kernel, dim3((unsigned)sgrid), dim3(256), 0, st, d, n, info, ticket_pre, part,
+                       (int64_t)grid * I8_T * 128, co_counter, colmax, (int)m, sigma, rscale, history);
     TM_LAUNCH_CHECK();
     prof_begin(st);
     auto go = [&](auto kern) {
@@ -713,16 +731,12 @@
     prof_end(st);
     TM_LAUNCH_CHECK();
     hipLaunchKernelGGL(syrk_i8_finish_kernel, dim3(I8_T, 4), dim3(64, 16), 0, st, part, grid, (int)m, rscale, info,
-                       out, ldo);
-    hipLaunchKernelGGL(i8_envelope_kernel, dim3(1), dim3(I8_W), 0, st, out, ldo, colmax, (int)m, n, info, history);
+                       out, ldo, colmax, n, history, ticket_fin);
     TM_LAUNCH_CHECK();
     prof_hold(true);
-    rc = run_syrk_co_flagged(X, ldx, n, m, d, out, ldo, colsum, &info->flag, wb + own_bytes, st, center, v, xtv);
+    rc = run_syrk_co_flagged(X, ldx, n, m, d, out, ldo, colsum, &info->flag, wb + own_bytes, st, center, v, xtv,
+                             history != nullptr ? reinterpret_cast<double *>(history + 4) : nullptr);
     prof_hold(false);
-    if (rc == TM_OK && history != nullptr) {
-        hipLaunchKernelGGL(i8_record_diag_kernel, dim3(1), dim3(I8_W), 0, st, out, ldo, (int)m, history);
-        TM_LAUNCH_CHECK();
-    }
     return rc;
 }
 
```

New measurement: 1058 GB/s. 1.3% lower.
